# deepomicslab/PALACE

Measured on AMD Instinct MI355X. Metric: contigs/sec eref+generate_graph+matching, 1M-contig synth, 1/2/4/8 GPU, higher is better.
Workload: dtype u32

## Files before the change

palace_amd/csrc/common.hpp:

```cpp
#pragma once
#include <hip/hip_runtime.h>
#include <cstdarg>
#include <cstdint>
#include <cstdio>
#include <cstring>
#include <vector>

#include "../../include/palace_hip.h"

namespace palace {

void set_error(const char *fmt, ...);

#define PALACE_HIP_TRY(expr)                                                                    \
    do {                                                                                        \
        hipError_t e__ = (expr);                                                                \
        if (e__ != hipSuccess) {                                                                \
            palace::set_error("%s failed: %s (%s:%d)", #expr, hipGetErrorString(e__), __FILE__, \
                              __LINE__);                                                        \
            return PALACE_EHIP;                                                                 \
        }                                                                                       \
    } while (0)

#define PALACE_REQUIRE(cond, msg)                                  \
    do {                                                           \
        if (!(cond)) {                                             \
            palace::set_error("%s: %s", __func__, msg);            \
            return PALACE_EINVAL;                                  \
        }                                                          \
    } while (0)

constexpr int kWave = 64;
constexpr int kCUs = 256;
constexpr size_t kPlaneBytes = 1ull << 29;
constexpr size_t kPlaneWords = 1ull << 27;

struct CoderMasks {
    uint32_t m[3][3];
};

struct Workspace {
    void *ptr = nullptr;
    size_t bytes = 0;
};

}

namespace palace {
struct MatchScratch;
void free_match_scratch(MatchScratch *m);
}

struct palace_ctx {
    int device = 0;
    hipStream_t stream = nullptr;
    bool owns_stream = true;
    hipEvent_t ev0 = nullptr, ev1 = nullptr;
    uint32_t key_buckets[4] = {~0u, ~0u, ~0u, ~0u};
    std::vector<hipEvent_t> marks;
    bool coder_set = false;
    palace::CoderMasks masks{};
    uint32_t *plane[3] = {nullptr, nullptr, nullptr};
    bool planes_external = false;
    bool want_final = false;
    bool final_only = false;
    bool table_clean = false;
    int64_t keys_counted = 0;
    const struct palace_eref_probe_index *probe_ix = nullptr;
    const struct palace_eref_probe_index *c0_hits_ix = nullptr;
    uint32_t hits_mask = 0;
    int probe_all_sets = 0;
    bool sent_scattered = false;
    int64_t scan_ref_lo = 0, scan_ref_hi = 0;
    const void *counts_ptr = nullptr;
    bool planeless = false;
    int count_mode = 0;
    int64_t bin_cap_override = 0;
    int64_t slab_override = 0;
    palace::Workspace ws;
    bool ws_grown = false;
    palace::Workspace pin;
    palace::MatchScratch *match_scratch = nullptr;
    int64_t graph_border = -1;
    const void *graph_border_cands = nullptr;
    int64_t graph_border_n = -1;
    int match_grid = 0;
    bool match_two_word_keys = false;
    int match_iters = 0;
    uint64_t *d_small = nullptr;
};

namespace palace {
int ensure_workspace(palace_ctx *ctx, size_t bytes);
int ensure_pinned(palace_ctx *ctx, size_t bytes);
int ensure_table(palace_ctx *ctx);
}
```

palace_amd/csrc/decomp.hip:

```cpp
#include "decomp.hpp"

#include <algorithm>

namespace palace {

namespace {

constexpr uint64_t kNoKey = ~0ull;
constexpr uint64_t kClosed = 0;
constexpr int kStampShift = 42;
constexpr int kPackedShift = 52, kPackedStamps = 1 << (64 - kPackedShift);
constexpr uint64_t kLenMask = (1ull << 40) - 1;


__device__ __forceinline__ uint64_t wave_incl_scan(uint64_t v, int lane)
{
#pragma unroll
    for (int d = 1; d < 64; d <<= 1) {
        const uint64_t u = __shfl_up(v, d);
        if (lane >= d) v += u;
    }
    return v;
}

constexpr int kMaxWaves = 16;

__device__ void scan_partials_body(const uint64_t *__restrict__ in, int64_t n, uint64_t *__restrict__ partials, int blk, int nblk)
{
    __shared__ uint64_t part[kMaxWaves];
    const int64_t chunk = (n + nblk - 1) / nblk;
    const int64_t a = min(n, static_cast<int64_t>(blk) * chunk), e = min(n, a + chunk);
    uint64_t s = 0;
    for (int64_t i = a + threadIdx.x; i < e; i += blockDim.x) s += in[i];
    const int lane = threadIdx.x & 63, waves = static_cast<int>(blockDim.x >> 6);
    s = wave_incl_scan(s, lane);
    if (lane == 63) part[threadIdx.x >> 6] = s;
    __syncthreads();
    if (threadIdx.x == 0) {
        uint64_t t = 0;
        for (int w = 0; w < waves; w++) t += part[w];
        partials[blk] = t;
    }
    __syncthreads();
}

__device__ void scan_prefix_body(uint64_t *__restrict__ partials, int n_parts, uint64_t *__restrict__ total)
{
    __shared__ uint64_t part[kMaxWaves];
    const int lane = threadIdx.x & 63, wv = threadIdx.x >> 6;
    const uint64_t x = static_cast<int>(threadIdx.x) < n_parts ? partials[threadIdx.x] : 0;
    const uint64_t incl = wave_incl_scan(x, lane);
    if (lane == 63) part[wv] = incl;
    __syncthreads();
    uint64_t before = 0;
    for (int w = 0; w < wv; w++) before += part[w];
    if (static_cast<int>(threadIdx.x) < n_parts) partials[threadIdx.x] = before + incl - x;
    if (threadIdx.x == blockDim.x - 1) *total = before + incl;
    __syncthreads();
}

__device__ void scan_apply_body(const uint64_t *__restrict__ in, uint64_t *__restrict__ out, int64_t n, const uint64_t *__restrict__ partials,
                                int blk, int nblk)
{
    __shared__ uint64_t part[kMaxWaves];
    const int64_t chunk = (n + nblk - 1) / nblk;
    const int64_t a = min(n, static_cast<int64_t>(blk) * chunk), e = min(n, a + chunk);
    const int lane = threadIdx.x & 63, wv = threadIdx.x >> 6, waves = static_cast<int>(blockDim.x >> 6);
    uint64_t carry = partials[blk];
    for (int64_t base = a; base < e; base += blockDim.x) {
        const int64_t i = base + threadIdx.x;
        const uint64_t x = i < e ? in[i] : 0;
        const uint64_t incl = wave_incl_scan(x, lane);
        if (lane == 63) part[wv] = incl;
        __syncthreads();
        uint64_t before = 0, all = 0;
        for (int w = 0; w < waves; w++) { if (w < wv) before += part[w]; all += part[w]; }
        if (i < e) out[i] = carry + before + incl - x;
        carry += all;
        __syncthreads();
    }
}

__global__ __launch_bounds__(kDecompBlock) void scan_partials_kernel(const uint64_t *__restrict__ in, const int32_t *__restrict__ n_dev,
                                                                     uint64_t *__restrict__ partials)
{
    scan_partials_body(in, *n_dev, partials, static_cast<int>(blockIdx.x), static_cast<int>(gridDim.x));
}
__global__ __launch_bounds__(kDecompBlock) void scan_prefix_kernel(uint64_t *__restrict__ partials, int n_parts, uint64_t *__restrict__ total)
{
    scan_prefix_body(partials, n_parts, total);
}
__global__ __launch_bounds__(kDecompBlock) void scan_apply_kernel(const uint64_t *__restrict__ in, uint64_t *__restrict__ out,
                                                                  const int32_t *__restrict__ n_dev, const uint64_t *__restrict__ partials)
{
    scan_apply_body(in, out, *n_dev, partials, static_cast<int>(blockIdx.x), static_cast<int>(gridDim.x));
}

struct Span { int tid, n; };
__device__ __forceinline__ Span whole_grid() { return Span{static_cast<int>(blockIdx.x * blockDim.x + threadIdx.x), static_cast<int>(gridDim.x * blockDim.x)}; }

__device__ void ph_init(const DecompBufs &b, Span T, int64_t comp_cap, int64_t vert_cap, int n_flags, int allow_packed)
{
    DecompState *st = b.st;
    const int V = st->V;
    for (int i = T.tid; i < V; i += T.n) { b.bo_hi[i] = kNoKey; b.bi_hi[i] = kNoKey; b.on_path[i] = 0; }
    for (int i = T.tid; i < n_flags; i += T.n) b.changed[i] = 0;
    if (T.tid == 0) {
        st->n_comp = 0; st->n_vert = 0; st->comp_cap = comp_cap; st->vert_cap = vert_cap;
        st->unsettled = 0; st->overflow = 0; st->bad = 0; st->dead = 0; st->scan_total = 0; st->alive_after = 0;
        st->packed = (allow_packed && b.kc && b.pack_bad && *b.pack_bad == 0) ? 1u : 0u;
        if (comp_cap >= 0) b.o_off[0] = 0;
    }
}

__device__ void ph_round_begin(const DecompBufs &b, Span T, int reset_left)
{
    const int V = b.st->V;
    if (!reset_left && b.st->dead) return;
    if (T.tid == 0) { b.st->alive_after = 0; if (reset_left) b.st->dead = 0; }
    const int64_t E = b.st->E;
    for (int64_t e = T.tid; e < E; e += T.n) b.done[e] = 0;
    const bool packed = b.st->packed != 0;
    for (int i = T.tid; i < V; i += T.n) {
        const int s = i >> 1;
        const int64_t l = reset_left ? 1 : b.left[s];
        if (reset_left && !(i & 1)) b.left[s] = 1;
        b.alive[i] = l > 0;
        b.next[i] = -1; b.prev[i] = -1;
        b.bo_hi[i] = b.bi_hi[i] = l > 0 ? kNoKey : kClosed;
        if (!packed) { b.bo_lo[i] = kNoKey; b.bo_lo[V + i] = kNoKey; b.bi_lo[i] = kNoKey; b.bi_lo[V + i] = kNoKey; }
        b.len_a[i] = 0;
    }
}

struct IterArgs {
    uint64_t stamp;
    uint64_t stamp_p;
    int parity;
    int prev_flag, flag;
    int unique_hi;
};


__device__ void ph_propose_hi(const DecompBufs &b, Span T, const IterArgs &a)
{
    if (b.st->dead) return;
    if (a.prev_flag >= 0 && !b.changed[a.prev_flag]) return;
    const int64_t E = b.st->E;
    const int V = b.st->V;
    const int other = (a.parity ^ 1) * V;
    const bool packed = b.st->packed != 0;
    for (int64_t e = T.tid; e < E; e += T.n) {
        if (b.done[e]) continue;
        const int u = b.src[e], v = b.dst[e];
        if (b.bi_hi[v] == kClosed) { b.done[e] = 1; continue; }
        const uint64_t k = packed ? (a.stamp_p | b.kc[e]) : (a.stamp | b.khi[e]);
        if (atomicMin(reinterpret_cast<unsigned long long *>(&b.bo_hi[u]), static_cast<unsigned long long>(k)) == kClosed) { b.done[e] = 1; continue; }
        atomicMin(reinterpret_cast<unsigned long long *>(&b.bi_hi[v]), static_cast<unsigned long long>(k));
        if (!a.unique_hi && !packed) { b.bo_lo[other + u] = kNoKey; b.bi_lo[other + v] = kNoKey; }
    }
}

__device__ void ph_propose_lo(const DecompBufs &b, Span T, const IterArgs &a)
{
    if (b.st->dead) return;
    if (a.prev_flag >= 0 && !b.changed[a.prev_flag]) return;
    if (b.st->packed) return;
    const int64_t E = b.st->E;
    const int mine = a.parity * b.st->V;
    for (int64_t e = T.tid; e < E; e += T.n) {
        if (b.done[e]) continue;
        const int u = b.src[e], v = b.dst[e];
        const uint64_t k = a.stamp | b.khi[e], lo = b.klo[e];
        if (b.bo_hi[u] == k) atomicMin(reinterpret_cast<unsigned long long *>(&b.bo_lo[mine + u]), static_cast<unsigned long long>(lo));
        if (b.bi_hi[v] == k) atomicMin(reinterpret_cast<unsigned long long *>(&b.bi_lo[mine + v]), static_cast<unsigned long long>(lo));
    }
}

__device__ void ph_commit_flag(const DecompBufs &b, Span T, const IterArgs &a, volatile unsigned int *took);
__device__ void ph_commit(const DecompBufs &b, Span T, const IterArgs &a)
{
    if (b.st->dead) return;
    if (a.prev_flag >= 0 && !b.changed[a.prev_flag]) return;
    ph_commit_flag(b, T, a, b.changed + a.flag);
}
__device__ void ph_commit_flag(const DecompBufs &b, Span T, const IterArgs &a, volatile unsigned int *took)
{
    bool any = false;
    const int64_t E = b.st->E;
    const int mine = a.parity * b.st->V;
    const bool packed = b.st->packed != 0;
    for (int64_t e = T.tid; e < E; e += T.n) {
        if (b.done[e]) continue;
        const int u = b.src[e], v = b.dst[e];
        const uint64_t k = packed ? (a.stamp_p | b.kc[e]) : (a.stamp | b.khi[e]);
        if (b.bo_hi[u] != k || b.bi_hi[v] != k) continue;
        const uint64_t lo = b.klo[e];
        if (!a.unique_hi && !packed && (b.bo_lo[mine + u] != lo || b.bi_lo[mine + v] != lo)) continue;
        b.next[u] = v; b.prev[v] = u;
        b.nhi[u] = b.khi[e]; b.nlo[u] = lo;
        b.bo_hi[u] = kClosed; b.bi_hi[v] = kClosed;
        b.done[e] = 1;
        any = true;
    }
    if (__syncthreads_or(any) && threadIdx.x == 0) *took = 1u;
}

__device__ void ph_heads(const DecompBufs &b, Span T, int round, int last_flag)
{
    DecompState *st = b.st;
    if (st->dead) return;
    if (T.tid == 0 && last_flag >= 0 && b.changed[last_flag]) st->unsettled = 1;
    const int V = st->V;
    for (int v = T.tid; v < V; v += T.n) {
        if (!b.alive[v] || b.prev[v] >= 0) continue;
        int len = 0, last = v;
        int64_t least = b.left[v >> 1];
        for (int x = v; x >= 0; x = b.next[x]) {
            b.on_path[x] = round + 1;
            last = x;
            len++;
            least = min(least, b.left[x >> 1]);
        }
        const int twin_first = last ^ 1;
        if (v > twin_first) continue;
        const int64_t uses = twin_first == v ? 2 : 1;
        b.len_a[v] = (1ull << 40) | static_cast<uint64_t>(len);
        b.pay[v] = max(static_cast<int64_t>(1), least / uses);
        b.kind[v] = 0;
        b.open_at[v] = 0;
    }
}

__device__ void ph_cycles(const DecompBufs &b, Span T, int round)
{
    const int V = b.st->V;
    if (b.st->dead) return;
    for (int v = T.tid; v < V; v += T.n) {
        if (!b.alive[v] || b.on_path[v] == round + 1) continue;
        int len = 1, twin_least = v ^ 1, worst = 0;
        uint64_t whi = b.nhi[v], wlo = b.nlo[v];
        int64_t least = b.left[v >> 1];
        bool first = true;
        for (int x = b.next[v]; x != v; x = b.next[x]) {
            if (x < v) { first = false; break; }
            twin_least = min(twin_least, x ^ 1);
            const uint64_t hi = b.nhi[x], lo = b.nlo[x];
            if (hi > whi || (hi == whi && lo > wlo)) { whi = hi; wlo = lo; worst = len; }
            least = min(least, b.left[x >> 1]);
            len++;
        }
        if (!first || v > twin_least) continue;
        const int64_t uses = twin_least == v ? 2 : 1;
        b.len_a[v] = (1ull << 40) | static_cast<uint64_t>(len);
        b.pay[v] = max(static_cast<int64_t>(1), least / uses);
        b.kind[v] = 1;
        b.open_at[v] = (worst + 1) % len;
    }
}

__device__ void ph_emit(const DecompBufs &b, Span T, int round, int64_t c0, int64_t v0)
{
    DecompState *st = b.st;
    const int V = st->V;
    if (st->dead) return;
    int64_t alive = 0;
    for (int v = T.tid; v < V; v += T.n) {
        const uint64_t la = b.len_a[v];
        if (!la) continue;
        const int64_t len = static_cast<int64_t>(la & kLenMask);
        const uint64_t p = b.pos[v];
        const int64_t c = c0 + static_cast<int64_t>(p >> 40), at = v0 + static_cast<int64_t>(p & kLenMask);
        const int64_t pay = b.pay[v];
        const bool room = c < st->comp_cap && at + len <= st->vert_cap;
        if (!room) st->overflow = 1;
        else { b.o_off[c] = at; b.o_kind[c] = b.kind[v]; b.o_iter[c] = round; b.o_open[c] = b.open_at[v]; }
        int x = v;
        int64_t still = 0;
        for (int64_t k = 0; k < len; k++) {
            if (room) b.o_verts[at + k] = 2 * b.orig[x >> 1] + (x & 1);
            const int64_t l = b.left[x >> 1];
            b.left[x >> 1] = max(static_cast<int64_t>(0), l - pay);
            still += l - pay > 0;
            x = b.next[x];
        }
        alive += still;
    }
    __shared__ unsigned long long wg_alive;
    if (threadIdx.x == 0) wg_alive = 0;
    __syncthreads();
    if (alive) atomicAdd(&wg_alive, static_cast<unsigned long long>(alive));
    __syncthreads();
    if (threadIdx.x == 0 && wg_alive) atomicAdd(reinterpret_cast<unsigned long long *>(&st->alive_after), wg_alive);
}


__global__ void dec_init_kernel(DecompBufs b, int64_t comp_cap, int64_t vert_cap, int n_flags, int allow_packed) { ph_init(b, whole_grid(), comp_cap, vert_cap, n_flags, allow_packed); }
__global__ void dec_round_begin_kernel(DecompBufs b, int reset_left) { ph_round_begin(b, whole_grid(), reset_left); }
__global__ void dec_propose_hi_kernel(DecompBufs b, IterArgs a) { ph_propose_hi(b, whole_grid(), a); }
__global__ void dec_propose_lo_kernel(DecompBufs b, IterArgs a) { ph_propose_lo(b, whole_grid(), a); }
__global__ void dec_commit_kernel(DecompBufs b, IterArgs a) { ph_commit(b, whole_grid(), a); }
__global__ void dec_heads_kernel(DecompBufs b, int round, int last_flag) { ph_heads(b, whole_grid(), round, last_flag); }
__global__ void dec_cycles_kernel(DecompBufs b, int round) { ph_cycles(b, whole_grid(), round); }
__global__ void dec_emit_kernel(DecompBufs b, int round) { ph_emit(b, whole_grid(), round, b.st->n_comp, b.st->n_vert); }

__global__ void dec_round_end_kernel(DecompBufs b)
{
    DecompState *st = b.st;
    if (blockIdx.x || threadIdx.x || st->dead) return;
    st->dead = st->alive_after == 0;
    st->n_comp += static_cast<int64_t>(st->scan_total >> 40);
    st->n_vert += static_cast<int64_t>(st->scan_total & kLenMask);
    if (st->n_comp <= st->comp_cap) b.o_off[st->n_comp] = st->n_vert;
}

size_t up256(size_t v) { return (v + 255) / 256 * 256; }

struct Carver {
    char *base;
    size_t used = 0;
    template <class T>
    T *take(size_t n)
    {
        T *p = base ? reinterpret_cast<T *>(base + used) : nullptr;
        used += up256(std::max<size_t>(1, n) * sizeof(T));
        return p;
    }
};

size_t carve_all(DecompBufs &b, char *base, int64_t s_cap, int64_t e_cap, int64_t comp_cap, int64_t vert_cap, int rounds, int iters)
{
    Carver c{base};
    const size_t S = static_cast<size_t>(std::max<int64_t>(1, s_cap)), V = 2 * S, E = static_cast<size_t>(std::max<int64_t>(1, e_cap));
    b.st = c.take<DecompState>(1);
    b.src = c.take<int32_t>(E); b.dst = c.take<int32_t>(E);
    b.khi = c.take<uint64_t>(E); b.klo = c.take<uint64_t>(E);
    b.done = c.take<uint8_t>(E);
    b.kc = c.take<uint64_t>(E);
    b.left = c.take<int64_t>(S); b.orig = c.take<int32_t>(S);
    b.next = c.take<int32_t>(V); b.prev = c.take<int32_t>(V); b.on_path = c.take<int32_t>(V); b.open_at = c.take<int32_t>(V);
    b.nhi = c.take<uint64_t>(V); b.nlo = c.take<uint64_t>(V);
    b.bo_hi = c.take<uint64_t>(V); b.bi_hi = c.take<uint64_t>(V);
    b.bo_lo = c.take<uint64_t>(2 * V); b.bi_lo = c.take<uint64_t>(2 * V);
    b.len_a = c.take<uint64_t>(V); b.pos = c.take<uint64_t>(V);
    b.pay = c.take<int64_t>(V);
    b.alive = c.take<uint8_t>(V); b.kind = c.take<uint8_t>(V);
    b.partials = c.take<uint64_t>(kDecompGrid + 1);
    b.changed = c.take<uint32_t>(static_cast<size_t>(rounds) * static_cast<size_t>(iters));
    b.o_off = c.take<int64_t>(static_cast<size_t>(comp_cap) + 1);
    b.o_verts = c.take<int32_t>(static_cast<size_t>(vert_cap));
    b.o_iter = c.take<int32_t>(static_cast<size_t>(comp_cap));
    b.o_open = c.take<int32_t>(static_cast<size_t>(comp_cap));
    b.o_kind = c.take<uint8_t>(static_cast<size_t>(comp_cap));
    return c.used;
}

}

size_t decomp_bytes(int64_t s_cap, int64_t e_cap, int64_t comp_cap, int64_t vert_cap, int rounds, int iters)
{
    DecompBufs tmp;
    return carve_all(tmp, nullptr, s_cap, e_cap, comp_cap, vert_cap, rounds, iters);
}

void decomp_carve(DecompBufs &b, char *base, int64_t s_cap, int64_t e_cap, int64_t comp_cap, int64_t vert_cap, int rounds, int iters)
{
    carve_all(b, base, s_cap, e_cap, comp_cap, vert_cap, rounds, iters);
}

int scan_u64(palace_ctx *ctx, const uint64_t *in, uint64_t *out, const int32_t *n_dev, uint64_t *partials, uint64_t *total_dev)
{
    hipLaunchKernelGGL(scan_partials_kernel, dim3(kDecompGrid), dim3(kDecompBlock), 0, ctx->stream, in, n_dev, partials);
    hipLaunchKernelGGL(scan_prefix_kernel, dim3(1), dim3(kDecompBlock), 0, ctx->stream, partials, kDecompGrid, total_dev);
    hipLaunchKernelGGL(scan_apply_kernel, dim3(kDecompGrid), dim3(kDecompBlock), 0, ctx->stream, in, out, n_dev, partials);
    PALACE_HIP_TRY(hipGetLastError());
    return PALACE_OK;
}

namespace {

const dim3 kBlock(kDecompBlock);
constexpr int kWideGridDefault = 2048;
inline dim3 wide_grid(const palace_ctx *ctx) { return dim3(ctx->match_grid > 0 ? ctx->match_grid : kWideGridDefault); }

void enqueue_iterations(palace_ctx *ctx, const DecompBufs &b, int first, int n, uint64_t *count, int flag0, bool unique_hi)
{
    for (int k = 0; k < n; k++) {
        IterArgs a{((1ull << 21) - 1 - *count) << kStampShift, static_cast<uint64_t>((kPackedStamps - 1 - *count) & (kPackedStamps - 1)) << kPackedShift,
                   (first + k) & 1, k ? flag0 + k - 1 : -1, flag0 + k, unique_hi ? 1 : 0};
        (*count)++;
        hipLaunchKernelGGL(dec_propose_hi_kernel, wide_grid(ctx), kBlock, 0, ctx->stream, b, a);
        if (!unique_hi) hipLaunchKernelGGL(dec_propose_lo_kernel, wide_grid(ctx), kBlock, 0, ctx->stream, b, a);
        hipLaunchKernelGGL(dec_commit_kernel, wide_grid(ctx), kBlock, 0, ctx->stream, b, a);
    }
}

int enqueue_read_off(palace_ctx *ctx, const DecompBufs &b, int round, int last_flag)
{
    hipLaunchKernelGGL(dec_heads_kernel, wide_grid(ctx), kBlock, 0, ctx->stream, b, round, last_flag);
    hipLaunchKernelGGL(dec_cycles_kernel, wide_grid(ctx), kBlock, 0, ctx->stream, b, round);
    int rc = scan_u64(ctx, b.len_a, b.pos, &b.st->V, b.partials, &b.st->scan_total);
    if (rc) return rc;
    hipLaunchKernelGGL(dec_emit_kernel, wide_grid(ctx), kBlock, 0, ctx->stream, b, round);
    hipLaunchKernelGGL(dec_round_end_kernel, dim3(1), dim3(64), 0, ctx->stream, b);
    PALACE_HIP_TRY(hipGetLastError());
    return PALACE_OK;
}

}

int decomp_begin(palace_ctx *ctx, const DecompBufs &b, int rounds, int64_t comp_cap, int64_t vert_cap)
{
    PALACE_REQUIRE(rounds >= 1 && rounds <= kMaxRounds, "round count out of range");
    static_assert(kDecompGrid <= kDecompBlock, "scan_prefix_kernel scans the block sums with one workgroup");
    const int allow_packed = !ctx->match_two_word_keys && static_cast<int64_t>(rounds) * kMaxIters < kPackedStamps ? 1 : 0;
    hipLaunchKernelGGL(dec_init_kernel, wide_grid(ctx), kBlock, 0, ctx->stream, b, comp_cap, vert_cap, rounds * kMaxIters, allow_packed);
    PALACE_HIP_TRY(hipGetLastError());
    return PALACE_OK;
}

int decomp_rounds(palace_ctx *ctx, const DecompBufs &b, int t0, int t1, int rounds, int aggressive, int iters, bool unique_hi,
                  uint64_t *count)
{
    PALACE_REQUIRE(0 <= t0 && t0 <= t1 && t1 <= rounds && rounds <= kMaxRounds && iters >= 1 && iters <= kMaxIters, "round / iteration count out of range");
    for (int t = t0; t < t1; t++) {
        hipLaunchKernelGGL(dec_round_begin_kernel, wide_grid(ctx), kBlock, 0, ctx->stream, b, (aggressive && t == rounds - 1) ? 1 : 0);
        enqueue_iterations(ctx, b, 0, iters, count, t * kMaxIters, unique_hi);
        int rc = enqueue_read_off(ctx, b, t, t * kMaxIters + iters - 1);
        if (rc) return rc;
    }
    PALACE_HIP_TRY(hipGetLastError());
    return PALACE_OK;
}

int decomp_run_checked(palace_ctx *ctx, const DecompBufs &b, int rounds, int aggressive, bool unique_hi, int64_t comp_cap,
                       int64_t vert_cap, int64_t max_iterations)
{
    PALACE_REQUIRE(rounds >= 1 && rounds <= kMaxRounds, "round count out of range");
    constexpr int kBatch = 16;
    hipLaunchKernelGGL(dec_init_kernel, wide_grid(ctx), kBlock, 0, ctx->stream, b, comp_cap, vert_cap, kBatch, 0);
    uint64_t count = 0;
    for (int t = 0; t < rounds; t++) {
        hipLaunchKernelGGL(dec_round_begin_kernel, wide_grid(ctx), kBlock, 0, ctx->stream, b, (aggressive && t == rounds - 1) ? 1 : 0);
        for (int first = 0;; first += kBatch) {
            PALACE_HIP_TRY(hipMemsetAsync(b.changed, 0, kBatch * sizeof(uint32_t), ctx->stream));
            enqueue_iterations(ctx, b, first, kBatch, &count, 0, unique_hi);
            uint32_t last = 0;
            PALACE_HIP_TRY(hipMemcpyAsync(&last, b.changed + kBatch - 1, sizeof last, hipMemcpyDeviceToHost, ctx->stream));
            PALACE_HIP_TRY(hipStreamSynchronize(ctx->stream));
            if (!last) break;
            if (static_cast<int64_t>(count) > max_iterations || count + kBatch >= (1ull << 21)) {
                set_error("matching: no fixed point after %llu iterations", static_cast<unsigned long long>(count));
                return PALACE_ESTATE;
            }
        }
        PALACE_HIP_TRY(hipMemsetAsync(b.changed, 0, kBatch * sizeof(uint32_t), ctx->stream));
        int rc = enqueue_read_off(ctx, b, t, kBatch - 1);
        if (rc) return rc;
    }
    return PALACE_OK;
}

int decomp_group(palace_ctx *ctx, const DecompBufs &b, DecompRun &run, int rounds, int aggressive, bool unique_hi)
{
    const int first = kFirstGroupRounds;
    const int t0 = run.next_round, t1 = std::min(rounds, t0 + (t0 == 0 ? first : kRoundsPerGroup));
    for (int t = t0; t < t1; t++) {
        const int iters = ctx->match_iters > 0 ? std::min(ctx->match_iters, kMaxIters) : (t == 0 ? kFirstRoundIters : kLaterRoundIters);
        int rc = decomp_rounds(ctx, b, t, t + 1, rounds, aggressive, iters, unique_hi, &run.count);
        if (rc) return rc;
    }
    run.next_round = t1;
    return PALACE_OK;
}

int decomp_finish(palace_ctx *ctx, const DecompBufs &b, DecompRun &run, int rounds, int aggressive, bool unique_hi, int64_t comp_cap,
                  int64_t vert_cap, int64_t max_iterations, DecompState *h_state, const std::function<int()> &reset_left)
{
    for (;;) {
        PALACE_HIP_TRY(hipMemcpyAsync(h_state, b.st, sizeof *h_state, hipMemcpyDeviceToHost, ctx->stream));
        PALACE_HIP_TRY(hipStreamSynchronize(ctx->stream));
        if (h_state->unsettled) {
            int rc = reset_left();
            if (rc) return rc;
            rc = decomp_run_checked(ctx, b, rounds, aggressive, unique_hi, comp_cap, vert_cap, max_iterations);
            if (rc) return rc;
            PALACE_HIP_TRY(hipMemcpyAsync(h_state, b.st, sizeof *h_state, hipMemcpyDeviceToHost, ctx->stream));
            PALACE_HIP_TRY(hipStreamSynchronize(ctx->stream));
            return PALACE_OK;
        }
        if (run.next_round >= rounds) return PALACE_OK;
        if (h_state->alive_after == 0) {
            if (!aggressive) return PALACE_OK;
            run.next_round = rounds - 1;
        }
        int rc = decomp_group(ctx, b, run, rounds, aggressive, unique_hi);
        if (rc) return rc;
    }
}

}
```

palace_amd/csrc/decomp.hpp:

```cpp
#pragma once
#include <functional>

#include "common.hpp"

struct palace_match_result {
    int64_t n = 0;
    int64_t *off = nullptr;
    int32_t *verts = nullptr, *iter = nullptr, *open_at = nullptr;
    uint8_t *kind = nullptr;
    uint64_t *bare = nullptr;
    int64_t n_bare = 0;
    bool borrowed = false;
    ~palace_match_result();
};

namespace palace {

constexpr int kDecompGrid = 256;
constexpr int kDecompBlock = 256;
constexpr int kMaxRounds = 1024;
constexpr int kMaxIters = 64;

struct DecompState {
    int32_t S, V;
    int64_t E;
    int64_t n_comp, n_vert;
    int64_t comp_cap, vert_cap;
    uint32_t unsettled;
    uint32_t overflow;
    uint32_t bad;
    uint32_t dead;
    uint32_t packed;
    uint64_t scan_total;
    int64_t alive_after;
};

struct DecompBufs {
    DecompState *st = nullptr;
    int32_t *src = nullptr, *dst = nullptr;
    uint64_t *khi = nullptr, *klo = nullptr;
    uint8_t *done = nullptr;
    uint64_t *kc = nullptr;
    const uint32_t *pack_bad = nullptr;
    int64_t *left = nullptr;
    int32_t *orig = nullptr;
    int32_t *next = nullptr, *prev = nullptr, *on_path = nullptr, *open_at = nullptr;
    uint64_t *nhi = nullptr, *nlo = nullptr;
    uint64_t *bo_hi = nullptr, *bi_hi = nullptr;
    uint64_t *bo_lo = nullptr, *bi_lo = nullptr;
    uint64_t *len_a = nullptr, *pos = nullptr;
    int64_t *pay = nullptr;
    uint8_t *alive = nullptr, *kind = nullptr;
    uint64_t *partials = nullptr;
    uint32_t *changed = nullptr;
    int64_t *o_off = nullptr;
    int32_t *o_verts = nullptr, *o_iter = nullptr, *o_open = nullptr;
    uint8_t *o_kind = nullptr;
};

size_t decomp_bytes(int64_t s_cap, int64_t e_cap, int64_t comp_cap, int64_t vert_cap, int rounds, int iters);
void decomp_carve(DecompBufs &b, char *base, int64_t s_cap, int64_t e_cap, int64_t comp_cap, int64_t vert_cap, int rounds, int iters);
constexpr int kFirstRoundIters = 7, kLaterRoundIters = 4, kRoundsPerGroup = 5, kFirstGroupRounds = 5;
int decomp_begin(palace_ctx *ctx, const DecompBufs &b, int rounds, int64_t comp_cap, int64_t vert_cap);
int decomp_rounds(palace_ctx *ctx, const DecompBufs &b, int t0, int t1, int rounds, int aggressive, int iters, bool unique_hi,
                  uint64_t *count);

struct DecompRun { int next_round = 0; uint64_t count = 0; };
int decomp_group(palace_ctx *ctx, const DecompBufs &b, DecompRun &run, int rounds, int aggressive, bool unique_hi);
int decomp_finish(palace_ctx *ctx, const DecompBufs &b, DecompRun &run, int rounds, int aggressive, bool unique_hi, int64_t comp_cap,
                  int64_t vert_cap, int64_t max_iterations, DecompState *h_state, const std::function<int()> &reset_left);

int decomp_run_checked(palace_ctx *ctx, const DecompBufs &b, int rounds, int aggressive, bool unique_hi, int64_t comp_cap,
                       int64_t vert_cap, int64_t max_iterations);

int scan_u64(palace_ctx *ctx, const uint64_t *in, uint64_t *out, const int32_t *n_dev, uint64_t *partials, uint64_t *total_dev);

}
```

palace_amd/csrc/filter.hip:

```cpp
#include <algorithm>
#include <cstdlib>
#include <memory>
#include <vector>

#include "common.hpp"
#include "decomp.hpp"

namespace palace {
namespace {

constexpr uint64_t kEmptyKey = ~0ull;
constexpr uint64_t kWeightTop = 1ull << 40;

struct FilterState {
    int32_t n_segs, S_f, n_sel, n_resc;
    int64_t n_edges, n_junc, n_kept2, n_kept3, n_arcs;
    int64_t n_static, n_dyn;
    int64_t n_path_arcs;
    uint32_t bad, pack_bad;
    uint64_t scan_total;
};
enum : uint32_t { kBadPathToken = 1, kBadNoSeg = 2, kBadEdgeBound = 4, kBadArcTable = 8 };

struct ArcTable {
    uint64_t *key;
    unsigned long long *w;
    uint32_t *backed;
    uint64_t mask;
    int64_t *list, list_cap;
};

struct PathArcs {
    uint64_t *key;
    int32_t *idx;
    uint64_t mask;
    int32_t *u, *v;
    int32_t *arc_of;
    int64_t n, cap;
};

struct F {
    FilterState *fs;
    int32_t n_segs, min_count;
    const uint8_t *seed;
    const int32_t *tlen, *rank, *name_len;
    int32_t *by_rank;
    int64_t n_paths;
    const int64_t *path_off;
    const int32_t *path_tok;
    uint8_t *core, *sel, *near, *resc, *seg_flags, *edge_flags, *has_arc;
    int32_t *fid, *contig_of;
    uint64_t *scan_in, *scan_out;
    int64_t edge_bound;
    ArcTable t;
    PathArcs pa;
    int32_t *arc_u, *arc_v;
    unsigned long long *arc_w;
    uint8_t *arc_backed;
    int64_t arc_cap;
    int use_paths;
    uint64_t *bare;
};

__device__ __forceinline__ int gtid() { return static_cast<int>(blockIdx.x * blockDim.x + threadIdx.x); }
__device__ __forceinline__ int gsize() { return static_cast<int>(gridDim.x * blockDim.x); }

__global__ void st4_by_rank_kernel(F f)
{
    for (int s = gtid(); s < f.n_segs; s += gsize()) f.by_rank[f.rank[s]] = s;
}

__global__ void st4_begin_kernel(F f, const int64_t *__restrict__ d_n_edges, int64_t call_bound)
{
    for (int s = gtid(); s < f.n_segs; s += gsize()) {
        const uint8_t c = f.seed[s] != 0 && f.tlen[s] > 0;
        f.core[s] = c; f.sel[s] = c; f.near[s] = 0; f.resc[s] = 0;
    }
    if (gtid() == 0) {
        FilterState *fs = f.fs;
        const int64_t n = *d_n_edges;
        fs->n_segs = f.n_segs; fs->S_f = 0; fs->n_sel = 0; fs->n_resc = 0;
        const int64_t bound = call_bound < f.edge_bound ? call_bound : f.edge_bound;
        fs->n_edges = n < 0 ? 0 : (n > bound ? bound : n);
        fs->n_junc = 0; fs->n_kept2 = 0; fs->n_kept3 = 0; fs->n_arcs = 0; fs->n_static = 0; fs->n_dyn = 0;
        fs->bad = n > bound ? kBadEdgeBound : 0u;
        fs->pack_bad = 0;
        fs->scan_total = 0;
    }
}

__device__ __forceinline__ int64_t edge_total(const palace_graph_edge &e)
{
    return static_cast<int64_t>(e.counts[0]) + e.counts[1] + e.counts[2] + e.counts[3];
}

__global__ void st4_pass2_kernel(F f, const palace_graph_edge *__restrict__ edges)
{
    const int64_t n = f.fs->n_edges;
    int64_t juncs = 0, kept = 0;
    for (int64_t i = gtid(); i < n; i += gsize()) {
        const palace_graph_edge e = edges[i];
        uint8_t fl = 0;
        if (edge_total(e) >= f.min_count) {
            fl = 1; juncs++;
            if (e.left == e.right || f.core[e.left] || f.core[e.right]) {
                fl |= 2; kept++;
                f.near[e.left] = 1; f.near[e.right] = 1;
                f.sel[e.left] = 1; f.sel[e.right] = 1;
            }
        }
        f.edge_flags[i] = fl;
    }
    if (juncs) atomicAdd(reinterpret_cast<unsigned long long *>(&f.fs->n_junc), static_cast<unsigned long long>(juncs));
    if (kept) atomicAdd(reinterpret_cast<unsigned long long *>(&f.fs->n_kept2), static_cast<unsigned long long>(kept));
}

__global__ void st4_pass3_kernel(F f, const palace_graph_edge *__restrict__ edges)
{
    const int64_t n = f.fs->n_edges;
    int64_t kept = 0;
    for (int64_t i = gtid(); i < n; i += gsize()) {
        const uint8_t fl = f.edge_flags[i];
        if (!(fl & 1)) continue;
        const palace_graph_edge e = edges[i];
        if (f.core[e.left] || f.near[e.left] || f.core[e.right] || f.near[e.right]) {
            f.edge_flags[i] = fl | 4;
            if (!(fl & 2)) kept++;
            f.sel[e.left] = 1; f.sel[e.right] = 1;
        }
    }
    if (kept) atomicAdd(reinterpret_cast<unsigned long long *>(&f.fs->n_kept3), static_cast<unsigned long long>(kept));
}

__global__ void st4_paths_kernel(F f)
{
    for (int64_t p = gtid(); p < f.n_paths; p += gsize()) {
        const int64_t a = f.path_off[p], b = f.path_off[p + 1];
        int64_t total = 0, backed = 0;
        bool known = true;
        for (int64_t k = a; k < b; k++) {
            const int32_t t = f.path_tok[k];
            if (t < 0) { known = false; break; }
            const int32_t m = t >> 1;
            total += f.name_len[m];
            if (f.seed[m]) backed += f.name_len[m];
        }
        if (!known) { atomicOr(&f.fs->bad, kBadPathToken); continue; }
        if (backed > 0 && (static_cast<double>(backed) / static_cast<double>(total) >= 0.5 || backed > 2000))
            for (int64_t k = a; k < b; k++) f.resc[f.path_tok[k] >> 1] = 1;
    }
}

__global__ void st4_order_kernel(F f)
{
    for (int r = gtid(); r < f.n_segs; r += gsize()) {
        const int s = f.by_rank[r];
        const bool sel = f.sel[s], resc = f.resc[s] && !sel;
        if (resc && f.tlen[s] <= 0) atomicOr(&f.fs->bad, kBadNoSeg);
        f.scan_in[r] = (sel ? (1ull << 32) : 0ull) | (resc ? 1ull : 0ull);
    }
}

__global__ void st4_ids_kernel(F f)
{
    FilterState *fs = f.fs;
    const int32_t n_sel = static_cast<int32_t>(fs->scan_total >> 32), n_resc = static_cast<int32_t>(fs->scan_total & 0xffffffffu);
    for (int r = gtid(); r < f.n_segs; r += gsize()) {
        const int s = f.by_rank[r];
        const uint64_t in = f.scan_in[r], before = f.scan_out[r];
        int32_t id = -1;
        if (in >> 32) id = static_cast<int32_t>(before >> 32);
        else if (in & 1) id = n_sel + static_cast<int32_t>(before & 0xffffffffu);
        f.fid[s] = id;
        if (id >= 0) { f.contig_of[id] = s; f.has_arc[id] = 0; }
        f.seg_flags[s] = static_cast<uint8_t>((in >> 32 ? 1 : 0) | (in & 1 ? 2 : 0) | (f.core[s] ? 4 : 0));
    }
    if (gtid() == 0) { fs->n_sel = n_sel; fs->n_resc = n_resc; fs->S_f = n_sel + n_resc; }
}

__device__ __forceinline__ uint64_t mix(uint64_t x)
{
    x ^= x >> 33; x *= 0xff51afd7ed558ccdull; x ^= x >> 33; x *= 0xc4ceb9fe1a85ec53ull; x ^= x >> 33;
    return x;
}

__device__ void path_arc_insert(const F &f, int32_t u, int32_t v)
{
    const PathArcs &pa = f.pa;
    const uint64_t key = (static_cast<uint64_t>(static_cast<uint32_t>(u)) << 32) | static_cast<uint32_t>(v);
    uint64_t s = mix(key) & pa.mask;
    for (uint64_t probes = 0; probes <= pa.mask; probes++) {
        const uint64_t cur = pa.key[s];
        if (cur == key) return;
        if (cur == kEmptyKey) {
            const uint64_t old = atomicCAS(reinterpret_cast<unsigned long long *>(&pa.key[s]), kEmptyKey, key);
            if (old == kEmptyKey) {
                const int64_t at = static_cast<int64_t>(atomicAdd(reinterpret_cast<unsigned long long *>(&f.fs->n_path_arcs), 1ull));
                if (at < pa.cap) { pa.u[at] = u; pa.v[at] = v; pa.idx[s] = static_cast<int32_t>(at); }
                return;
            }
            if (old == key) return;
        }
        s = (s + 1) & pa.mask;
    }
}
__global__ void st4_path_arcs_kernel(F f)
{
    for (int64_t p = gtid(); p < f.n_paths; p += gsize()) {
        int32_t before = -1;
        for (int64_t k = f.path_off[p]; k < f.path_off[p + 1]; k++) {
            const int32_t here = f.path_tok[k];
            if (before >= 0 && here >= 0) {
                path_arc_insert(f, before, here);
                if ((here ^ 1) != before) path_arc_insert(f, here ^ 1, before ^ 1);
            }
            before = here;
        }
    }
}
__device__ __forceinline__ int32_t path_arc_find(const PathArcs &pa, int32_t u, int32_t v)
{
    const uint64_t key = (static_cast<uint64_t>(static_cast<uint32_t>(u)) << 32) | static_cast<uint32_t>(v);
    uint64_t s = mix(key) & pa.mask;
    for (;;) {
        const uint64_t cur = pa.key[s];
        if (cur == key) return pa.idx[s];
        if (cur == kEmptyKey) return -1;
        s = (s + 1) & pa.mask;
    }
}

__global__ __launch_bounds__(kDecompBlock) void st4_arcs_static_kernel(F f)
{
    __shared__ uint32_t wave_n[kDecompBlock / 64];
    __shared__ long long block_base;
    const PathArcs &pa = f.pa;
    const int lane = threadIdx.x & 63, wave = threadIdx.x >> 6;
    for (int64_t p0 = static_cast<int64_t>(blockIdx.x) * blockDim.x; p0 < pa.n; p0 += static_cast<int64_t>(gridDim.x) * blockDim.x) {
        const int64_t p = p0 + threadIdx.x;
        int32_t fu = -1, fv = -1;
        if (p < pa.n) {
            const int32_t cu = pa.u[p] >> 1, cv = pa.v[p] >> 1;
            if ((f.seg_flags[cu] & 3) && (f.seg_flags[cv] & 3)) { fu = f.fid[cu]; fv = f.fid[cv]; }
        }
        const bool in = fu >= 0 && fv >= 0;
        const unsigned long long m = __ballot(in);
        if (lane == 0) wave_n[wave] = static_cast<uint32_t>(__popcll(m));
        __syncthreads();
        if (threadIdx.x == 0) {
            uint32_t total = 0;
            for (int w = 0; w < kDecompBlock / 64; w++) { const uint32_t c = wave_n[w]; wave_n[w] = total; total += c; }
            block_base = total ? static_cast<long long>(atomicAdd(reinterpret_cast<unsigned long long *>(&f.fs->n_static), static_cast<unsigned long long>(total))) : 0ll;
        }
        __syncthreads();
        if (p < pa.n) {
            int32_t at = -1;
            if (in) {
                const int64_t slot = block_base + wave_n[wave] + __popcll(m & ((1ull << lane) - 1));
                if (slot < f.arc_cap) {
                    at = static_cast<int32_t>(slot);
                    f.arc_u[at] = 2 * fu + (pa.u[p] & 1); f.arc_v[at] = 2 * fv + (pa.v[p] & 1);
                    f.arc_w[at] = 0; f.arc_backed[at] = 1;
                } else atomicOr(&f.fs->bad, kBadArcTable);
            }
            pa.arc_of[p] = at;
        }
        __syncthreads();
    }
}

__device__ void bump_arc(const F &f, int32_t cu, int32_t cv, int32_t u, int32_t v, int64_t w)
{
    if (f.use_paths) {
        const int32_t p = path_arc_find(f.pa, cu, cv);
        if (p >= 0) {
            const int32_t at = f.pa.arc_of[p];
            if (at >= 0) { atomicAdd(&f.arc_w[at], static_cast<unsigned long long>(w)); return; }
        }
    }
    const ArcTable &t = f.t;
    const uint64_t key = (static_cast<uint64_t>(static_cast<uint32_t>(u)) << 32) | static_cast<uint32_t>(v);
    uint64_t s = mix(key) & t.mask;
    for (uint64_t probes = 0;; probes++) {
        if (probes > t.mask) { atomicOr(&f.fs->bad, kBadArcTable); return; }
        const uint64_t cur = t.key[s];
        if (cur == key) break;
        if (cur == kEmptyKey) {
            const uint64_t old = atomicCAS(reinterpret_cast<unsigned long long *>(&t.key[s]), kEmptyKey, key);
            if (old == kEmptyKey) {
                const int64_t at = static_cast<int64_t>(atomicAdd(reinterpret_cast<unsigned long long *>(&f.fs->n_dyn), 1ull));
                if (at < t.list_cap) t.list[at] = static_cast<int64_t>(s);
                else atomicOr(&f.fs->bad, kBadArcTable);
                break;
            }
            if (old == key) break;
        }
        s = (s + 1) & t.mask;
    }
    if (w) atomicAdd(&t.w[s], static_cast<unsigned long long>(w));
}

__global__ void st4_arcs_juncs_kernel(F f, const palace_graph_edge *__restrict__ edges)
{
    const int64_t n = f.fs->n_edges;
    for (int64_t i = gtid(); i < n; i += gsize()) {
        if (!(f.edge_flags[i] & 6)) continue;
        const palace_graph_edge e = edges[i];
        const int64_t w = min(edge_total(e), static_cast<int64_t>(kWeightTop - 1));
        const int32_t cu = 2 * e.left + (e.oL & 1), cv = 2 * e.right + (e.oR & 1);
        const int32_t u = 2 * f.fid[e.left] + (e.oL & 1), v = 2 * f.fid[e.right] + (e.oR & 1);
        bump_arc(f, cu, cv, u, v, w);
        if ((v ^ 1) != u) bump_arc(f, cv ^ 1, cu ^ 1, v ^ 1, u ^ 1, w);
    }
}

__global__ void st4_arcs_dyn_kernel(F f)
{
    FilterState *fs = f.fs;
    const int64_t n_static = min(fs->n_static, f.arc_cap), n = min(fs->n_dyn, f.t.list_cap);
    for (int64_t a = gtid(); a < n; a += gsize()) {
        const int64_t s = f.t.list[a];
        const uint64_t key = f.t.key[s];
        const int64_t at = n_static + a;
        if (at < f.arc_cap) {
            f.arc_u[at] = static_cast<int32_t>(key >> 32); f.arc_v[at] = static_cast<int32_t>(key & 0xffffffffu);
            f.arc_w[at] = f.t.w[s]; f.arc_backed[at] = 0;
        } else atomicOr(&fs->bad, kBadArcTable);
        f.t.key[s] = kEmptyKey; f.t.w[s] = 0;
    }
    if (gtid() == 0) fs->n_arcs = min(n_static + n, f.arc_cap);
}

__global__ void st4_arc_keys_kernel(F f, DecompBufs b)
{
    const int64_t n = min(f.fs->n_static, f.arc_cap) + min(f.fs->n_dyn, f.t.list_cap);
    for (int64_t a = gtid(); a < n && a < f.arc_cap; a += gsize()) {
        const int32_t u = f.arc_u[a], v = f.arc_v[a];
        const uint64_t w = min(static_cast<uint64_t>(f.arc_w[a]), kWeightTop - 1);
        b.khi[a] = ((kWeightTop - w) << 1) | (f.arc_backed[a] ? 0u : 1u);
        const uint64_t key = (static_cast<uint64_t>(static_cast<uint32_t>(u)) << 32) | static_cast<uint32_t>(v);
        const uint64_t twin = (static_cast<uint64_t>(static_cast<uint32_t>(v ^ 1)) << 32) | static_cast<uint32_t>(u ^ 1);
        const uint64_t cls = min(key, twin);
        b.klo[a] = (cls << 1) | (key != cls ? 1u : 0u);
        f.has_arc[u >> 1] = 1; f.has_arc[v >> 1] = 1;
    }
}

__global__ void st4_sub_in_kernel(F f)
{
    const int n = f.fs->S_f;
    for (int i = gtid(); i < n; i += gsize()) f.scan_in[i] = f.has_arc[i];
}

__global__ void st4_sub_kernel(F f, DecompBufs b, const int32_t *__restrict__ cn)
{
    FilterState *fs = f.fs;
    const int n = fs->S_f;
    const int32_t n_sub = static_cast<int32_t>(fs->scan_total);
    for (int i = gtid(); i < n; i += gsize()) {
        if (!f.has_arc[i]) continue;
        const int32_t sub = static_cast<int32_t>(f.scan_out[i]);
        b.orig[sub] = i;
        b.left[sub] = max(1, cn[f.contig_of[i]]);
    }
    const int64_t n_arcs = min(fs->n_arcs, f.arc_cap);
    const int vbits = 32 - __clz(max(1, 2 * n_sub - 1)), wbits = min(40, 51 - 2 * vbits);
    const uint64_t wmax = wbits > 0 ? (1ull << wbits) - 1 : 0;
    if (gtid() == 0 && wbits <= 0) fs->pack_bad = 1;
    for (int64_t a = gtid(); a < n_arcs; a += gsize()) {
        const int32_t u = f.arc_u[a], v = f.arc_v[a];
        const int32_t su = 2 * static_cast<int32_t>(f.scan_out[u >> 1]) + (u & 1), sv = 2 * static_cast<int32_t>(f.scan_out[v >> 1]) + (v & 1);
        b.src[a] = su;
        b.dst[a] = sv;
        if (wbits > 0) {
            const uint64_t w = f.arc_w[a];
            if (w > wmax) atomicOr(&fs->pack_bad, 1u);
            const uint64_t key = (static_cast<uint64_t>(su) << vbits) | static_cast<uint32_t>(sv);
            const uint64_t twin = (static_cast<uint64_t>(sv ^ 1) << vbits) | static_cast<uint32_t>(su ^ 1);
            b.kc[a] = ((wmax - min(w, wmax)) << (2 * vbits + 1)) | (static_cast<uint64_t>(f.arc_backed[a] ? 0u : 1u) << (2 * vbits)) | min(key, twin);
        }
    }
    if (gtid() == 0) { b.st->S = n_sub; b.st->V = 2 * n_sub; b.st->E = n_arcs; }
}

__global__ void st4_left_kernel(F f, DecompBufs b, const int32_t *__restrict__ cn)
{
    const int n = f.fs->S_f;
    for (int i = gtid(); i < n; i += gsize())
        if (f.has_arc[i]) b.left[static_cast<int32_t>(f.scan_out[i])] = max(1, cn[f.contig_of[i]]);
}

__global__ void st4_bare_kernel(F f)
{
    const int n = f.fs->S_f, words = (n + 63) / 64;
    for (int w = gtid(); w < words; w += gsize()) {
        uint64_t bits = 0;
        for (int k = 0; k < 64 && w * 64 + k < n; k++)
            if (!f.has_arc[w * 64 + k]) bits |= 1ull << k;
        f.bare[w] = bits;
    }
}

size_t up(size_t v) { return (v + 255) / 256 * 256; }
uint64_t pow2_at_least(uint64_t v) { uint64_t p = 1024; while (p < v) p <<= 1; return p; }

template <class T>
T *carve(char *&p, size_t n)
{
    T *r = reinterpret_cast<T *>(p);
    p += up(std::max<size_t>(1, n) * sizeof(T));
    return r;
}

}
}

struct palace_stage04 {
    palace::F f{};
    palace::DecompBufs b{};
    char *fixed = nullptr;
    char *grown = nullptr;
    size_t grown_bytes = 0;
    int64_t n_tok = 0, edge_bound = 0, s_cap = 0, e_cap = 0, comp_cap = 0, vert_cap = 0;
    int rounds = 0, aggressive = 0, last_rounds = 0;
    palace::DecompRun run;
    bool filtered = false, matched = false;
    const int32_t *d_cn = nullptr;
    char *pin = nullptr;
    size_t pin_bytes = 0;
    palace::FilterState *h_fs = nullptr;
    palace::DecompState *h_ds = nullptr;
    palace_match_result res;
    int32_t *h_contig_of = nullptr;
};

using namespace palace;

namespace {

const dim3 kG(1024), kB(kDecompBlock);

int grow_pinned(palace_ctx *ctx, palace_stage04 *s, size_t bytes)
{
    if (s->pin_bytes >= bytes) return PALACE_OK;
    if (s->pin) { PALACE_HIP_TRY(hipStreamSynchronize(ctx->stream)); PALACE_HIP_TRY(hipHostFree(s->pin)); s->pin = nullptr; s->pin_bytes = 0; }
    const size_t want = bytes + bytes / 4 + (1 << 16);
    hipError_t e = hipHostMalloc(reinterpret_cast<void **>(&s->pin), want, hipHostMallocDefault);
    if (e != hipSuccess) { set_error("stage04: hipHostMalloc(%zu) failed: %s", want, hipGetErrorString(e)); return PALACE_ENOMEM; }
    s->pin_bytes = want;
    return PALACE_OK;
}

int grow_device(palace_ctx *ctx, palace_stage04 *s, int64_t edge_bound, int rounds)
{
    const int64_t e_dyn = 2 * edge_bound + 16;
    const int64_t e_cap = e_dyn + s->f.pa.n + 16;
    const int64_t s_cap = std::min<int64_t>(s->f.n_segs, e_cap);
    const int64_t comp_cap = static_cast<int64_t>(rounds) * s_cap + 16, vert_cap = 2 * comp_cap;
    const uint64_t slots = pow2_at_least(2 * static_cast<uint64_t>(e_dyn));
    const size_t dec = decomp_bytes(s_cap, e_cap, comp_cap, vert_cap, rounds, kMaxIters);
    const size_t bytes = up(static_cast<size_t>(edge_bound) + 1) + up(slots * 8) * 2 + up(static_cast<size_t>(e_dyn) * 8) +
                         2 * up(static_cast<size_t>(e_cap) * 4) + up(static_cast<size_t>(e_cap) * 8) + up(static_cast<size_t>(e_cap)) + dec + 8192;
    if (s->grown_bytes < bytes || s->edge_bound < edge_bound || s->rounds < rounds) {
        if (s->grown) { PALACE_HIP_TRY(hipStreamSynchronize(ctx->stream)); PALACE_HIP_TRY(hipFree(s->grown)); s->grown = nullptr; s->grown_bytes = 0; }
        hipError_t e = hipMalloc(reinterpret_cast<void **>(&s->grown), bytes);
        if (e != hipSuccess) { set_error("stage04: hipMalloc(%zu) failed: %s", bytes, hipGetErrorString(e)); return PALACE_ENOMEM; }
        s->grown_bytes = bytes;
        char *p = s->grown;
        s->f.edge_flags = carve<uint8_t>(p, static_cast<size_t>(edge_bound) + 1);
        s->f.t.key = carve<uint64_t>(p, slots);
        s->f.t.w = carve<unsigned long long>(p, slots);
        s->f.t.backed = nullptr;
        s->f.t.mask = slots - 1;
        s->f.t.list = carve<int64_t>(p, static_cast<size_t>(e_dyn));
        s->f.t.list_cap = e_dyn;
        s->f.arc_u = carve<int32_t>(p, static_cast<size_t>(e_cap));
        s->f.arc_v = carve<int32_t>(p, static_cast<size_t>(e_cap));
        s->f.arc_w = carve<unsigned long long>(p, static_cast<size_t>(e_cap));
        s->f.arc_backed = carve<uint8_t>(p, static_cast<size_t>(e_cap));
        s->f.arc_cap = e_cap;
        decomp_carve(s->b, p, s_cap, e_cap, comp_cap, vert_cap, rounds, kMaxIters);
        s->b.pack_bad = &s->f.fs->pack_bad;
        PALACE_HIP_TRY(hipMemsetAsync(s->f.t.key, 0xff, slots * 8, ctx->stream));
        PALACE_HIP_TRY(hipMemsetAsync(s->f.t.w, 0, slots * 8, ctx->stream));
        s->edge_bound = edge_bound; s->s_cap = s_cap; s->e_cap = e_cap; s->comp_cap = comp_cap; s->vert_cap = vert_cap; s->rounds = rounds;
    }
    s->f.edge_bound = s->edge_bound;
    return PALACE_OK;
}

}

extern "C" {

int palace_stage04_create(palace_ctx *ctx, const palace_stage04_inputs *in, palace_stage04 **out)
{
    PALACE_REQUIRE(ctx && in && out, "null argument");
    PALACE_REQUIRE(in->n_segs >= 0 && in->n_segs < (1 << 30) && in->n_paths >= 0 && in->min_count >= 0, "bad size");
    PALACE_REQUIRE(in->n_segs == 0 || (in->seed && in->tlen && in->rank && in->name_len), "null per-contig array");
    PALACE_REQUIRE(in->n_paths == 0 || (in->path_off && in->path_tok), "null path arrays");
    PALACE_HIP_TRY(hipSetDevice(ctx->device));
    const size_t n = static_cast<size_t>(in->n_segs);
    const int64_t n_tok = in->n_paths ? in->path_off[in->n_paths] : 0;
    PALACE_REQUIRE(n_tok >= 0 && (in->n_paths == 0 || in->path_off[0] == 0), "path offsets must start at 0 and ascend");
    int64_t n_pairs = 0;
    for (int64_t k = 0; k < in->n_paths; k++) {
        const int64_t len = in->path_off[k + 1] - in->path_off[k];
        PALACE_REQUIRE(len >= 0 && in->path_off[k + 1] <= n_tok, "path offsets must start at 0 and ascend");
        n_pairs += len > 1 ? len - 1 : 0;
    }
    for (int32_t i = 0; i < in->n_segs; i++) PALACE_REQUIRE(in->rank[i] >= 0 && in->rank[i] < in->n_segs, "rank out of range");
    for (int64_t k = 0; k < n_tok; k++) PALACE_REQUIRE(in->path_tok[k] < 2 * static_cast<int64_t>(in->n_segs), "path token out of range");
    std::unique_ptr<palace_stage04> s(new palace_stage04());
    const int64_t pa_cap = 2 * n_pairs + 16;
    const uint64_t pa_slots = pow2_at_least(2 * static_cast<uint64_t>(pa_cap));
    const size_t bytes = up(sizeof(FilterState)) + up(n) * 8 + up(n * 4) * 6 + up(n * 8) * 2 + up((static_cast<size_t>(in->n_paths) + 1) * 8) +
                         up(static_cast<size_t>(n_tok) * 4 + 4) + up((n + 63) / 64 * 8 + 8) + up(pa_slots * 8) + up(pa_slots * 4) +
                         3 * up(static_cast<size_t>(pa_cap) * 4) + 16384;
    hipError_t e = hipMalloc(reinterpret_cast<void **>(&s->fixed), bytes);
    if (e != hipSuccess) { set_error("stage04: hipMalloc(%zu) failed: %s", bytes, hipGetErrorString(e)); return PALACE_ENOMEM; }
    char *p = s->fixed;
    F &f = s->f;
    f.fs = carve<FilterState>(p, 1);
    f.n_segs = in->n_segs; f.min_count = in->min_count; f.n_paths = in->n_paths;
    uint8_t *seed = carve<uint8_t>(p, n);
    f.core = carve<uint8_t>(p, n); f.sel = carve<uint8_t>(p, n); f.near = carve<uint8_t>(p, n); f.resc = carve<uint8_t>(p, n);
    f.seg_flags = carve<uint8_t>(p, n); f.has_arc = carve<uint8_t>(p, n);
    int32_t *tlen = carve<int32_t>(p, n), *rank = carve<int32_t>(p, n), *name_len = carve<int32_t>(p, n);
    f.by_rank = carve<int32_t>(p, n); f.fid = carve<int32_t>(p, n); f.contig_of = carve<int32_t>(p, n);
    f.scan_in = carve<uint64_t>(p, n); f.scan_out = carve<uint64_t>(p, n);
    int64_t *path_off = carve<int64_t>(p, static_cast<size_t>(in->n_paths) + 1);
    int32_t *path_tok = carve<int32_t>(p, static_cast<size_t>(n_tok) + 1);
    f.bare = carve<uint64_t>(p, (n + 63) / 64 + 1);
    f.pa.key = carve<uint64_t>(p, pa_slots); f.pa.idx = carve<int32_t>(p, pa_slots); f.pa.mask = pa_slots - 1;
    f.pa.u = carve<int32_t>(p, static_cast<size_t>(pa_cap)); f.pa.v = carve<int32_t>(p, static_cast<size_t>(pa_cap));
    f.pa.arc_of = carve<int32_t>(p, static_cast<size_t>(pa_cap));
    f.pa.cap = pa_cap; f.pa.n = 0;
    f.seed = seed; f.tlen = tlen; f.rank = rank; f.name_len = name_len; f.path_off = path_off; f.path_tok = path_tok;
    s->n_tok = n_tok;
    auto fail = [&](hipError_t err) {
        set_error("stage04: upload failed: %s", hipGetErrorString(err));
        (void)hipFree(s->fixed);
        return PALACE_EHIP;
    };
    hipStream_t st = ctx->stream;
    if (n) {
        if ((e = hipMemcpyAsync(seed, in->seed, n, hipMemcpyHostToDevice, st)) != hipSuccess) return fail(e);
        if ((e = hipMemcpyAsync(tlen, in->tlen, n * 4, hipMemcpyHostToDevice, st)) != hipSuccess) return fail(e);
        if ((e = hipMemcpyAsync(rank, in->rank, n * 4, hipMemcpyHostToDevice, st)) != hipSuccess) return fail(e);
        if ((e = hipMemcpyAsync(name_len, in->name_len, n * 4, hipMemcpyHostToDevice, st)) != hipSuccess) return fail(e);
    }
    if (in->n_paths) {
        if ((e = hipMemcpyAsync(path_off, in->path_off, (static_cast<size_t>(in->n_paths) + 1) * 8, hipMemcpyHostToDevice, st)) != hipSuccess) return fail(e);
        if (n_tok && (e = hipMemcpyAsync(path_tok, in->path_tok, static_cast<size_t>(n_tok) * 4, hipMemcpyHostToDevice, st)) != hipSuccess) return fail(e);
    } else if ((e = hipMemsetAsync(path_off, 0, 8, st)) != hipSuccess) return fail(e);
    hipLaunchKernelGGL(st4_by_rank_kernel, kG, kB, 0, st, f);
    if ((e = hipMemsetAsync(f.fs, 0, sizeof(FilterState), st)) != hipSuccess) return fail(e);
    if ((e = hipMemsetAsync(f.pa.key, 0xff, pa_slots * 8, st)) != hipSuccess) return fail(e);
    hipLaunchKernelGGL(st4_path_arcs_kernel, kG, kB, 0, st, f);
    FilterState h_fs{};
    if ((e = hipMemcpyAsync(&h_fs, f.fs, sizeof h_fs, hipMemcpyDeviceToHost, st)) != hipSuccess) return fail(e);
    if ((e = hipStreamSynchronize(st)) != hipSuccess) return fail(e);
    if (h_fs.n_path_arcs > pa_cap) { (void)hipFree(s->fixed); set_error("stage04: path arc table too small"); return PALACE_ESTATE; }
    f.pa.n = h_fs.n_path_arcs;
    e = hipHostMalloc(reinterpret_cast<void **>(&s->h_fs), up(sizeof(FilterState)) + up(sizeof(DecompState)), hipHostMallocDefault);
    if (e != hipSuccess) { (void)hipFree(s->fixed); set_error("stage04: hipHostMalloc failed: %s", hipGetErrorString(e)); return PALACE_ENOMEM; }
    s->h_ds = reinterpret_cast<DecompState *>(reinterpret_cast<char *>(s->h_fs) + up(sizeof(FilterState)));
    s->res.borrowed = true;
    *out = s.release();
    return PALACE_OK;
}

int palace_stage04_destroy(palace_ctx *ctx, palace_stage04 *s)
{
    if (!s) return PALACE_OK;
    if (ctx) { (void)hipSetDevice(ctx->device); (void)hipStreamSynchronize(ctx->stream); }
    if (s->fixed) (void)hipFree(s->fixed);
    if (s->grown) (void)hipFree(s->grown);
    if (s->pin) (void)hipHostFree(s->pin);
    if (s->h_fs) (void)hipHostFree(s->h_fs);
    delete s;
    return PALACE_OK;
}

int palace_stage04_reserve(palace_ctx *ctx, palace_stage04 *s, int64_t edge_bound)
{
    PALACE_REQUIRE(ctx && s && edge_bound >= 0, "bad argument");
    PALACE_HIP_TRY(hipSetDevice(ctx->device));
    return grow_device(ctx, s, std::max<int64_t>(edge_bound, s->edge_bound), std::max(s->rounds, 11));
}

int palace_stage04_filter(palace_ctx *ctx, palace_stage04 *s, const palace_graph_edge *d_edges, const int64_t *d_n_edges,
                          int64_t edge_bound)
{
    PALACE_REQUIRE(ctx && s && d_n_edges && edge_bound >= 0, "bad argument");
    PALACE_REQUIRE(edge_bound == 0 || d_edges, "null edge array");
    PALACE_HIP_TRY(hipSetDevice(ctx->device));
    int rc = grow_device(ctx, s, std::max<int64_t>(edge_bound, s->edge_bound), std::max(s->rounds, 11));
    if (rc) return rc;
    rc = [&]() -> int {
        const F &f = s->f;
        hipStream_t st = ctx->stream;
        hipLaunchKernelGGL(st4_begin_kernel, kG, kB, 0, st, f, d_n_edges, edge_bound);
        hipLaunchKernelGGL(st4_pass2_kernel, kG, kB, 0, st, f, d_edges);
        hipLaunchKernelGGL(st4_pass3_kernel, kG, kB, 0, st, f, d_edges);
        hipLaunchKernelGGL(st4_paths_kernel, kG, kB, 0, st, f);
        hipLaunchKernelGGL(st4_order_kernel, kG, kB, 0, st, f);
        PALACE_HIP_TRY(hipGetLastError());
        int rc2 = scan_u64(ctx, f.scan_in, f.scan_out, &f.fs->n_segs, s->b.partials, &f.fs->scan_total);
        if (rc2) return rc2;
        hipLaunchKernelGGL(st4_ids_kernel, kG, kB, 0, st, f);
        PALACE_HIP_TRY(hipGetLastError());
        return PALACE_OK;
    }();
    if (rc) return rc;
    s->filtered = true;
    s->matched = false;
    return PALACE_OK;
}

static int enqueue_match(palace_ctx *ctx, palace_stage04 *s, const palace_graph_edge *d_edges, bool use_paths)
{
    s->f.use_paths = use_paths ? 1 : 0;
    const F &f = s->f;
    hipStream_t st = ctx->stream;
    if (use_paths) hipLaunchKernelGGL(st4_arcs_static_kernel, kG, kB, 0, st, f);
    hipLaunchKernelGGL(st4_arcs_juncs_kernel, kG, kB, 0, st, f, d_edges);
    hipLaunchKernelGGL(st4_arcs_dyn_kernel, kG, kB, 0, st, f);
    hipLaunchKernelGGL(st4_arc_keys_kernel, kG, kB, 0, st, f, s->b);
    hipLaunchKernelGGL(st4_sub_in_kernel, kG, kB, 0, st, f);
    PALACE_HIP_TRY(hipGetLastError());
    int rc = scan_u64(ctx, f.scan_in, f.scan_out, &f.fs->S_f, s->b.partials, &f.fs->scan_total);
    if (rc) return rc;
    hipLaunchKernelGGL(st4_sub_kernel, kG, kB, 0, st, f, s->b, s->d_cn);
    hipLaunchKernelGGL(st4_bare_kernel, kG, kB, 0, st, f);
    PALACE_HIP_TRY(hipGetLastError());
    return PALACE_OK;
}

int palace_stage04_match(palace_ctx *ctx, palace_stage04 *s, const palace_graph_edge *d_edges, const int32_t *d_cn,
                         int32_t iterations, int32_t aggressive, int32_t use_paths)
{
    PALACE_REQUIRE(ctx && s && d_cn && iterations >= 1, "bad argument");
    PALACE_REQUIRE(s->filtered, "palace_stage04_filter has not run");
    const int rounds = iterations + (aggressive ? 1 : 0);
    PALACE_REQUIRE(rounds <= kMaxRounds, "too many iterations");
    PALACE_REQUIRE(rounds <= s->rounds, "more rounds than the filter call reserved room for (at most 10 iterations + aggressive)");
    PALACE_HIP_TRY(hipSetDevice(ctx->device));
    s->d_cn = d_cn; s->aggressive = aggressive ? 1 : 0;
    s->f.use_paths = use_paths ? 1 : 0;
    int rc = enqueue_match(ctx, s, d_edges, use_paths != 0);
    if (rc) return rc;
    s->run = DecompRun{};
    if ((rc = decomp_begin(ctx, s->b, rounds, s->comp_cap, s->vert_cap))) return rc;
    if ((rc = decomp_group(ctx, s->b, s->run, rounds, s->aggressive, false))) return rc;
    PALACE_HIP_TRY(hipMemcpyAsync(s->h_fs, s->f.fs, sizeof(FilterState), hipMemcpyDeviceToHost, ctx->stream));
    s->rounds = std::max(s->rounds, rounds);
    s->matched = true;
    s->last_rounds = rounds;
    return PALACE_OK;
}

static int check_filter_state(const FilterState &fs)
{
    if (fs.bad & kBadPathToken) { set_error("stage04: contigs.paths names an unknown contig id (filter_graph.py:138 raises)"); return PALACE_EINVAL; }
    if (fs.bad & kBadNoSeg) { set_error("stage04: contigs.paths rescues a contig without SEG line (filter_graph.py:257 raises)"); return PALACE_EINVAL; }
    if (fs.bad & kBadEdgeBound) { set_error("stage04: more edges on the device than the bound given to palace_stage04_filter"); return PALACE_EINVAL; }
    if (fs.bad & kBadArcTable) { set_error("stage04: arc table full"); return PALACE_ESTATE; }
    return PALACE_OK;
}

int palace_stage04_counts(palace_ctx *ctx, palace_stage04 *s, int64_t counts[8])
{
    PALACE_REQUIRE(ctx && s && counts && s->filtered, "bad argument");
    PALACE_HIP_TRY(hipMemcpyAsync(s->h_fs, s->f.fs, sizeof(FilterState), hipMemcpyDeviceToHost, ctx->stream));
    PALACE_HIP_TRY(hipStreamSynchronize(ctx->stream));
    const FilterState &fs = *s->h_fs;
    int rc = check_filter_state(fs);
    if (rc) return rc;
    counts[0] = fs.n_edges; counts[1] = fs.n_junc; counts[2] = fs.n_kept2; counts[3] = fs.n_kept3;
    counts[4] = fs.n_sel; counts[5] = fs.n_resc; counts[6] = s->matched ? fs.n_arcs : -1; counts[7] = fs.S_f;
    return PALACE_OK;
}

int palace_stage04_flags(palace_ctx *ctx, palace_stage04 *s, uint8_t *h_seg_flags, uint8_t *h_edge_flags, int64_t n_edges)
{
    PALACE_REQUIRE(ctx && s && s->filtered && n_edges >= 0 && n_edges <= s->edge_bound, "bad argument");
    if (h_seg_flags && s->f.n_segs)
        PALACE_HIP_TRY(hipMemcpyAsync(h_seg_flags, s->f.seg_flags, static_cast<size_t>(s->f.n_segs), hipMemcpyDeviceToHost, ctx->stream));
    if (h_edge_flags && n_edges)
        PALACE_HIP_TRY(hipMemcpyAsync(h_edge_flags, s->f.edge_flags, static_cast<size_t>(n_edges), hipMemcpyDeviceToHost, ctx->stream));
    PALACE_HIP_TRY(hipStreamSynchronize(ctx->stream));
    return PALACE_OK;
}

int palace_stage04_result(palace_ctx *ctx, palace_stage04 *s, palace_match_result **out, const int32_t **contig_of_out,
                          int64_t *n_segs_filtered_out)
{
    PALACE_REQUIRE(ctx && s && out, "null argument");
    PALACE_REQUIRE(s->matched, "palace_stage04_match has not run");
    PALACE_HIP_TRY(hipSetDevice(ctx->device));
    hipStream_t st = ctx->stream;
    const int rounds = s->last_rounds;
    auto reset_left = [&]() -> int {
        hipLaunchKernelGGL(st4_left_kernel, kG, kB, 0, st, s->f, s->b, s->d_cn);
        PALACE_HIP_TRY(hipGetLastError());
        return PALACE_OK;
    };
    int rc = decomp_finish(ctx, s->b, s->run, rounds, s->aggressive, false, s->comp_cap, s->vert_cap, 2 * s->e_cap + 64, s->h_ds, reset_left);
    if (rc) return rc;
    rc = check_filter_state(*s->h_fs);
    if (rc) return rc;
    const DecompState &ds = *s->h_ds;
    if (ds.overflow || ds.n_comp > s->comp_cap || ds.n_vert > s->vert_cap) { set_error("stage04: component arrays too small"); return PALACE_ESTATE; }
    const size_t nc = static_cast<size_t>(ds.n_comp), nv = static_cast<size_t>(ds.n_vert), sf = static_cast<size_t>(s->h_fs->S_f);
    const size_t words = (sf + 63) / 64;
    rc = grow_pinned(ctx, s, up((nc + 1) * 8) + up(nv * 4 + 4) + 2 * up(nc * 4 + 4) + up(nc + 1) + up(words * 8 + 8) + up(sf * 4 + 4));
    if (rc) return rc;
    char *p = s->pin;
    palace_match_result &r = s->res;
    r.off = carve<int64_t>(p, nc + 1); r.verts = carve<int32_t>(p, nv + 1); r.iter = carve<int32_t>(p, nc + 1);
    r.open_at = carve<int32_t>(p, nc + 1); r.kind = carve<uint8_t>(p, nc + 1); r.bare = carve<uint64_t>(p, words + 1);
    s->h_contig_of = carve<int32_t>(p, sf + 1);
    PALACE_HIP_TRY(hipMemcpyAsync(r.off, s->b.o_off, (nc + 1) * 8, hipMemcpyDeviceToHost, st));
    if (nv) PALACE_HIP_TRY(hipMemcpyAsync(r.verts, s->b.o_verts, nv * 4, hipMemcpyDeviceToHost, st));
    if (nc) {
        PALACE_HIP_TRY(hipMemcpyAsync(r.iter, s->b.o_iter, nc * 4, hipMemcpyDeviceToHost, st));
        PALACE_HIP_TRY(hipMemcpyAsync(r.open_at, s->b.o_open, nc * 4, hipMemcpyDeviceToHost, st));
        PALACE_HIP_TRY(hipMemcpyAsync(r.kind, s->b.o_kind, nc, hipMemcpyDeviceToHost, st));
    }
    if (words) PALACE_HIP_TRY(hipMemcpyAsync(r.bare, s->f.bare, words * 8, hipMemcpyDeviceToHost, st));
    if (sf) PALACE_HIP_TRY(hipMemcpyAsync(s->h_contig_of, s->f.contig_of, sf * 4, hipMemcpyDeviceToHost, st));
    PALACE_HIP_TRY(hipStreamSynchronize(st));
    r.n = static_cast<int64_t>(nc);
    r.n_bare = static_cast<int64_t>(sf) - ds.S;
    *out = &s->res;
    if (contig_of_out) *contig_of_out = s->h_contig_of;
    if (n_segs_filtered_out) *n_segs_filtered_out = static_cast<int64_t>(sf);
    return PALACE_OK;
}

}
```

palace_amd/csrc/match.hip:

```cpp
#include "common.hpp"
#include "decomp.hpp"
#include <algorithm>
#include <map>
#include <memory>
#include <mutex>
#include <numeric>
#include <thread>

namespace palace {

constexpr int32_t kNone = -1;

struct MatchArgs {
    int32_t n_vertices;
    int64_t n_arcs;
    const int32_t *src, *dst;
    const int64_t *out_off, *in_off;
    const int32_t *out_arcs, *in_arcs;
    const uint8_t *alive;
    int32_t *next, *prev, *next_arc, *want_out, *want_in;
    unsigned int *changed;
};

__global__ void match_propose_kernel(MatchArgs a)
{
    int32_t v = blockIdx.x * blockDim.x + threadIdx.x;
    if (v >= a.n_vertices) return;
    int32_t wo = kNone, wi = kNone;
    if (a.alive[v]) {
        if (a.next[v] == kNone)
            for (int64_t k = a.out_off[v]; k < a.out_off[v + 1]; k++) {
                int32_t e = a.out_arcs[k], h = a.dst[e];
                if (a.alive[h] && a.prev[h] == kNone) { wo = e; break; }
            }
        if (a.prev[v] == kNone)
            for (int64_t k = a.in_off[v]; k < a.in_off[v + 1]; k++) {
                int32_t e = a.in_arcs[k], t = a.src[e];
                if (a.alive[t] && a.next[t] == kNone) { wi = e; break; }
            }
    }
    a.want_out[v] = wo;
    a.want_in[v] = wi;
}

__global__ void match_commit_kernel(MatchArgs a)
{
    int32_t v = blockIdx.x * blockDim.x + threadIdx.x;
    if (v >= a.n_vertices) return;
    int32_t e = a.want_out[v];
    if (e == kNone) return;
    int32_t h = a.dst[e];
    if (a.want_in[h] != e) return;
    a.next[v] = h;
    a.prev[h] = v;
    a.next_arc[v] = e;
    *a.changed = 1u;
}

__global__ void match_init_kernel(MatchArgs a)
{
    int32_t v = blockIdx.x * blockDim.x + threadIdx.x;
    if (v >= a.n_vertices) return;
    a.next[v] = kNone; a.prev[v] = kNone; a.next_arc[v] = kNone;
}

}

using namespace palace;

constexpr int kRoundsPerCheck = 4;

static int enqueue_rounds(palace_ctx *ctx, const MatchArgs &a, int n)
{
    const unsigned blocks = static_cast<unsigned>((a.n_vertices + 255) / 256);
    PALACE_HIP_TRY(hipMemsetAsync(a.changed, 0, 4, ctx->stream));
    for (int k = 0; k < n; k++) {
        hipLaunchKernelGGL(match_propose_kernel, dim3(blocks), dim3(256), 0, ctx->stream, a);
        hipLaunchKernelGGL(match_commit_kernel, dim3(blocks), dim3(256), 0, ctx->stream, a);
    }
    PALACE_HIP_TRY(hipGetLastError());
    return PALACE_OK;
}

extern "C" int palace_match_greedy(palace_ctx *ctx, int32_t n_vertices, int64_t n_arcs, const int32_t *d_src,
                                   const int32_t *d_dst, const int64_t *d_out_off, const int32_t *d_out_arcs,
                                   const int64_t *d_in_off, const int32_t *d_in_arcs, const uint8_t *d_alive,
                                   int32_t *d_next, int32_t *d_prev, int32_t *d_next_arc, int32_t *rounds_out)
{
    PALACE_REQUIRE(ctx && n_vertices >= 0 && n_arcs >= 0, "bad argument");
    if (rounds_out) *rounds_out = 0;
    if (n_vertices == 0) return PALACE_OK;
    PALACE_REQUIRE(d_out_off && d_in_off && d_alive && d_next && d_prev && d_next_arc, "null device pointer");
    PALACE_REQUIRE(n_arcs == 0 || (d_src && d_dst && d_out_arcs && d_in_arcs), "null arc arrays");
    PALACE_REQUIRE(n_arcs < (1ll << 31), "arc ids must fit in int32");
    PALACE_HIP_TRY(hipSetDevice(ctx->device));
    int rc = ensure_workspace(ctx, static_cast<size_t>(n_vertices) * 8 + 256);
    if (rc) return rc;
    MatchArgs a{};
    a.n_vertices = n_vertices; a.n_arcs = n_arcs; a.src = d_src; a.dst = d_dst;
    a.out_off = d_out_off; a.in_off = d_in_off; a.out_arcs = d_out_arcs; a.in_arcs = d_in_arcs;
    a.alive = d_alive; a.next = d_next; a.prev = d_prev; a.next_arc = d_next_arc;
    a.want_out = static_cast<int32_t *>(ctx->ws.ptr);
    a.want_in = a.want_out + n_vertices;
    a.changed = reinterpret_cast<unsigned int *>(ctx->d_small);
    const unsigned blocks = static_cast<unsigned>((n_vertices + 255) / 256);
    hipLaunchKernelGGL(match_init_kernel, dim3(blocks), dim3(256), 0, ctx->stream, a);
    int rounds = 0;
    for (;;) {
        unsigned int changed = 0;
        rc = enqueue_rounds(ctx, a, kRoundsPerCheck);
        if (rc) return rc;
        PALACE_HIP_TRY(hipMemcpyAsync(&changed, ctx->d_small, 4, hipMemcpyDeviceToHost, ctx->stream));
        PALACE_HIP_TRY(hipStreamSynchronize(ctx->stream));
        rounds += kRoundsPerCheck;
        if (!changed) break;
        if (rounds > n_vertices + 2 + kRoundsPerCheck) { set_error("palace_match_greedy: no fixed point"); return PALACE_ESTATE; }
    }
    if (rounds_out) *rounds_out = rounds;
    return PALACE_OK;
}

struct SubResult {
    std::vector<int64_t> off{0};
    std::vector<int32_t> verts, iter, open_at;
    std::vector<uint8_t> kind;
};

namespace palace {

class BlockPool {
public:
    void *take(size_t bytes)
    {
        bytes = std::max<size_t>(bytes, 64);
        {
            std::lock_guard<std::mutex> g(mu_);
            for (size_t i = 0; i < free_.size(); i++)
                if (free_[i].second >= bytes && free_[i].second <= 2 * bytes + (1 << 20)) {
                    void *p = free_[i].first;
                    sizes_[p] = free_[i].second;
                    free_.erase(free_.begin() + i);
                    return p;
                }
        }
        void *p = std::malloc(bytes);
        if (p) { std::lock_guard<std::mutex> g(mu_); sizes_[p] = bytes; }
        return p;
    }
    void give(void *p)
    {
        if (!p) return;
        std::lock_guard<std::mutex> g(mu_);
        const size_t bytes = sizes_[p];
        sizes_.erase(p);
        if (free_.size() < 16) free_.emplace_back(p, bytes);
        else std::free(p);
    }

private:
    std::mutex mu_;
    std::vector<std::pair<void *, size_t>> free_;
    std::map<void *, size_t> sizes_;
};
static BlockPool g_result_pool;

struct MatchScratch {
    std::vector<int32_t> new_id, old_id, ssrc, sdst;
    std::vector<int64_t> sub_copies;
    std::vector<uint64_t> has_arc;
    SubResult sub;
};
void free_match_scratch(MatchScratch *m) { delete m; }

template <class T>
struct Borrowed {
    T &home;
    T v;
    explicit Borrowed(T &h) : home(h), v(std::move(h)) {}
    ~Borrowed() { home = std::move(v); }
    Borrowed(const Borrowed &) = delete;
    Borrowed &operator=(const Borrowed &) = delete;
};

__global__ void iota_keys_kernel(uint64_t *__restrict__ khi, uint64_t *__restrict__ klo, int64_t n)
{
    for (int64_t i = static_cast<int64_t>(blockIdx.x) * blockDim.x + threadIdx.x; i < n; i += static_cast<int64_t>(gridDim.x) * blockDim.x) {
        khi[i] = static_cast<uint64_t>(i);
        klo[i] = 0;
    }
}

}

palace_match_result::~palace_match_result()
{
    if (borrowed) return;
    for (void *p : {(void *)off, (void *)verts, (void *)iter, (void *)open_at, (void *)kind, (void *)bare}) palace::g_result_pool.give(p);
}

static int decompose_core(palace_ctx *ctx, int32_t n_segs, const int64_t *copies, const int32_t *orig, int64_t n_arcs,
                          const int32_t *src, const int32_t *dst, int32_t iterations, int32_t aggressive, SubResult *res)
{
    using namespace palace;
    const int64_t S = n_segs, E = n_arcs;
    const int rounds = iterations + (aggressive ? 1 : 0);
    PALACE_REQUIRE(rounds <= kMaxRounds, "too many iterations");
    int64_t live_rounds = 0;
    for (int64_t s = 0; s < S; s++) live_rounds += std::min<int64_t>(iterations, std::max<int64_t>(1, copies[s]));
    if (aggressive) live_rounds += S;
    const int64_t comp_cap = live_rounds, vert_cap = 2 * live_rounds;
    const size_t dev_bytes = decomp_bytes(S, E, comp_cap, vert_cap, rounds, kMaxIters);
    int rc = ensure_workspace(ctx, dev_bytes);
    if (rc) return rc;
    DecompBufs b;
    decomp_carve(b, static_cast<char *>(ctx->ws.ptr), S, E, comp_cap, vert_cap, rounds, kMaxIters);
    const size_t e4 = (static_cast<size_t>(E) * 4 + 255) / 256 * 256, s8 = (static_cast<size_t>(S) * 8 + 255) / 256 * 256,
                 s4 = (static_cast<size_t>(S) * 4 + 255) / 256 * 256;
    rc = ensure_pinned(ctx, 2 * e4 + s8 + s4 + 512);
    if (rc) return rc;
    char *pin = static_cast<char *>(ctx->pin.ptr);
    int32_t *p_src = reinterpret_cast<int32_t *>(pin), *p_dst = reinterpret_cast<int32_t *>(pin + e4);
    int64_t *p_left = reinterpret_cast<int64_t *>(pin + 2 * e4);
    int32_t *p_orig = reinterpret_cast<int32_t *>(pin + 2 * e4 + s8);
    DecompState *p_st = reinterpret_cast<DecompState *>(pin + 2 * e4 + s8 + s4);
    DecompState *p_back = p_st + 1;
    std::copy(src, src + E, p_src); std::copy(dst, dst + E, p_dst);
    for (int64_t s = 0; s < S; s++) p_left[s] = std::max<int64_t>(1, copies[s]);
    std::copy(orig, orig + S, p_orig);
    std::memset(p_st, 0, sizeof *p_st);
    p_st->S = n_segs; p_st->V = 2 * n_segs; p_st->E = E;
    hipStream_t st = ctx->stream;
    auto upload = [&]() -> int {
        PALACE_HIP_TRY(hipMemcpyAsync(b.st, p_st, sizeof *p_st, hipMemcpyHostToDevice, st));
        if (E) {
            PALACE_HIP_TRY(hipMemcpyAsync(b.src, p_src, static_cast<size_t>(E) * 4, hipMemcpyHostToDevice, st));
            PALACE_HIP_TRY(hipMemcpyAsync(b.dst, p_dst, static_cast<size_t>(E) * 4, hipMemcpyHostToDevice, st));
            hipLaunchKernelGGL(iota_keys_kernel, dim3(kDecompGrid), dim3(kDecompBlock), 0, st, b.khi, b.klo, E);
        }
        PALACE_HIP_TRY(hipMemcpyAsync(b.left, p_left, static_cast<size_t>(S) * 8, hipMemcpyHostToDevice, st));
        PALACE_HIP_TRY(hipMemcpyAsync(b.orig, p_orig, static_cast<size_t>(S) * 4, hipMemcpyHostToDevice, st));
        return PALACE_OK;
    };
    auto fail = [&](int code) { (void)hipStreamSynchronize(st); return code; };
    hipError_t e = hipSuccess;
    if ((rc = upload())) return fail(rc);
    if ((rc = decomp_begin(ctx, b, rounds, comp_cap, vert_cap))) return fail(rc);
    DecompRun run;
    if ((rc = decomp_group(ctx, b, run, rounds, aggressive, true))) return fail(rc);
    auto reset_left = [&]() -> int {
        PALACE_HIP_TRY(hipMemcpyAsync(b.left, p_left, static_cast<size_t>(S) * 8, hipMemcpyHostToDevice, st));
        return PALACE_OK;
    };
    if ((rc = decomp_finish(ctx, b, run, rounds, aggressive, true, comp_cap, vert_cap, 2 * E + 64, p_back, reset_left))) return fail(rc);
    if (p_back->overflow || p_back->n_comp > comp_cap || p_back->n_vert > vert_cap) {
        set_error("decompose: component arrays too small (%lld components, %lld vertices)", (long long)p_back->n_comp, (long long)p_back->n_vert);
        return PALACE_ESTATE;
    }
    const size_t nc = static_cast<size_t>(p_back->n_comp), nv = static_cast<size_t>(p_back->n_vert);
    res->off.resize(nc + 1); res->verts.resize(nv); res->iter.resize(nc); res->open_at.resize(nc); res->kind.resize(nc);
    e = hipMemcpyAsync(res->off.data(), b.o_off, (nc + 1) * 8, hipMemcpyDeviceToHost, st);
    if (e == hipSuccess && nv) e = hipMemcpyAsync(res->verts.data(), b.o_verts, nv * 4, hipMemcpyDeviceToHost, st);
    if (e == hipSuccess && nc) e = hipMemcpyAsync(res->iter.data(), b.o_iter, nc * 4, hipMemcpyDeviceToHost, st);
    if (e == hipSuccess && nc) e = hipMemcpyAsync(res->open_at.data(), b.o_open, nc * 4, hipMemcpyDeviceToHost, st);
    if (e == hipSuccess && nc) e = hipMemcpyAsync(res->kind.data(), b.o_kind, nc, hipMemcpyDeviceToHost, st);
    if (e == hipSuccess) e = hipStreamSynchronize(st);
    if (e != hipSuccess) { set_error("decompose: %s", hipGetErrorString(e)); return fail(PALACE_EHIP); }
    return PALACE_OK;
}

namespace {

void radix_by(const std::vector<uint64_t> &key, std::vector<uint32_t> &perm, std::vector<uint32_t> &tmp)
{
    const size_t n = perm.size();
    uint64_t all_or = 0, all_and = ~0ull;
    for (size_t i = 0; i < n; i++) { all_or |= key[i]; all_and &= key[i]; }
    const uint64_t varying = all_or ^ all_and;
    std::vector<uint32_t> hist(65536);
    for (int shift = 0; shift < 64; shift += 16) {
        if (((varying >> shift) & 0xffffu) == 0) continue;
        std::fill(hist.begin(), hist.end(), 0u);
        for (size_t i = 0; i < n; i++) hist[(key[perm[i]] >> shift) & 0xffffu]++;
        uint32_t run = 0;
        for (auto &h : hist) { const uint32_t c = h; h = run; run += c; }
        for (size_t i = 0; i < n; i++) tmp[hist[(key[perm[i]] >> shift) & 0xffffu]++] = perm[i];
        perm.swap(tmp);
    }
}

}

extern "C" {

int palace_match_arcs_from_edges(const int32_t *cn, int32_t n_segs, const palace_graph_edge *edges, int64_t n_edges,
                                 int32_t min_count, int64_t *copies, int32_t *src, int32_t *dst, int64_t *weight,
                                 int64_t *n_arcs_out)
{
    PALACE_REQUIRE(n_segs >= 0 && n_edges >= 0 && n_arcs_out, "bad argument");
    PALACE_REQUIRE(n_segs == 0 || (cn && copies), "null segment arrays");
    PALACE_REQUIRE(n_edges == 0 || (edges && src && dst && weight), "null edge arrays");
    PALACE_REQUIRE(n_segs < (1 << 30) && n_edges < (1ll << 30), "graph too large for int32 ids");
    for (int32_t s = 0; s < n_segs; s++) copies[s] = std::max(1, cn[s]);
    const uint64_t V = 2ull * static_cast<uint64_t>(n_segs);
    static thread_local std::vector<uint64_t> pair, m_pair, m_cls, m_wkey;
    static thread_local std::vector<int64_t> w, m_w;
    static thread_local std::vector<uint32_t> perm, tmp;
    pair.clear(); w.clear(); m_pair.clear(); m_w.clear();
    pair.reserve(2 * n_edges); w.reserve(2 * n_edges);
    for (int64_t e = 0; e < n_edges; e++) {
        const palace_graph_edge &x = edges[e];
        const int64_t tot = static_cast<int64_t>(x.counts[0]) + x.counts[1] + x.counts[2] + x.counts[3];
        if (tot < min_count) continue;
        PALACE_REQUIRE(x.left >= 0 && x.left < n_segs && x.right >= 0 && x.right < n_segs, "edge endpoint out of range");
        const uint64_t u = 2ull * x.left + (x.oL & 1), v = 2ull * x.right + (x.oR & 1);
        pair.push_back(u * V + v); w.push_back(tot);
        if ((v ^ 1) != u) { pair.push_back((v ^ 1) * V + (u ^ 1)); w.push_back(tot); }
    }
    const size_t n = pair.size();
    perm.resize(n); tmp.resize(n);
    std::iota(perm.begin(), perm.end(), 0u);
    radix_by(pair, perm, tmp);
    m_pair.reserve(n); m_w.reserve(n);
    for (size_t i = 0; i < n; i++) {
        if (!m_pair.empty() && m_pair.back() == pair[perm[i]]) m_w.back() += w[perm[i]];
        else { m_pair.push_back(pair[perm[i]]); m_w.push_back(w[perm[i]]); }
    }
    const size_t m = m_pair.size();
    int64_t w_max = 0;
    for (int64_t x : m_w) w_max = std::max(w_max, x);
    m_cls.resize(m); m_wkey.resize(m);
    for (size_t i = 0; i < m; i++) {
        const uint64_t u = m_pair[i] / V, v = m_pair[i] % V;
        m_cls[i] = std::min(m_pair[i], (v ^ 1) * V + (u ^ 1));
        m_wkey[i] = static_cast<uint64_t>(w_max - m_w[i]);
    }
    perm.resize(m); tmp.resize(m);
    std::iota(perm.begin(), perm.end(), 0u);
    radix_by(m_cls, perm, tmp);
    radix_by(m_wkey, perm, tmp);
    for (size_t i = 0; i < m; i++) {
        const uint64_t p = m_pair[perm[i]];
        src[i] = static_cast<int32_t>(p / V); dst[i] = static_cast<int32_t>(p % V); weight[i] = m_w[perm[i]];
    }
    *n_arcs_out = static_cast<int64_t>(m);
    return PALACE_OK;
}

int palace_match_set_option(palace_ctx *ctx, const char *name, int64_t value)
{
    PALACE_REQUIRE(ctx && name, "null argument");
    if (!std::strcmp(name, "iters_per_round")) {
        PALACE_REQUIRE(value >= 0 && value <= palace::kMaxIters, "iters_per_round out of range");
        ctx->match_iters = static_cast<int>(value);
    } else if (!std::strcmp(name, "one_word_keys")) {
        PALACE_REQUIRE(value == 0 || value == 1, "one_word_keys must be 0 or 1");
        ctx->match_two_word_keys = value == 0;
    } else if (!std::strcmp(name, "decomp_grid")) {
        PALACE_REQUIRE(value >= 0 && value <= 65536, "decomp_grid out of range");
        ctx->match_grid = static_cast<int>(value);
    } else {
        palace::set_error("palace_match_set_option: unknown option '%s'", name);
        return PALACE_EINVAL;
    }
    return PALACE_OK;
}

int palace_match_decompose(palace_ctx *ctx, int32_t n_segs, const int64_t *copies, int64_t n_arcs,
                           const int32_t *src, const int32_t *dst, int32_t iterations, int32_t aggressive,
                           palace_match_result **out)
{
    return palace_match_decompose_ex(ctx, n_segs, copies, n_arcs, src, dst, iterations, aggressive, 0, out);
}

int palace_match_decompose_ex(palace_ctx *ctx, int32_t n_segs, const int64_t *copies, int64_t n_arcs,
                              const int32_t *src, const int32_t *dst, int32_t iterations, int32_t aggressive,
                              int32_t compact, palace_match_result **out)
{
    PALACE_REQUIRE(ctx && out && n_segs >= 0 && n_arcs >= 0 && iterations >= 1, "bad argument");
    PALACE_REQUIRE(n_segs == 0 || copies, "null copies");
    PALACE_REQUIRE(n_arcs == 0 || (src && dst), "null arc arrays");
    PALACE_REQUIRE(n_segs < (1 << 30) && n_arcs < (1ll << 31), "graph too large for int32 ids");
    PALACE_HIP_TRY(hipSetDevice(ctx->device));
    const int32_t V = 2 * n_segs;
    for (int64_t e = 0; e < n_arcs; e++)
        PALACE_REQUIRE(src[e] >= 0 && src[e] < V && dst[e] >= 0 && dst[e] < V, "arc endpoint out of range");
    if (!ctx->match_scratch) ctx->match_scratch = new palace::MatchScratch();
    palace::MatchScratch &ms = *ctx->match_scratch;
    palace::Borrowed<std::vector<int32_t>> b_new(ms.new_id), b_old(ms.old_id), b_ssrc(ms.ssrc), b_sdst(ms.sdst);
    palace::Borrowed<std::vector<int64_t>> b_sc(ms.sub_copies);
    auto &new_id = b_new.v, &old_id = b_old.v, &ssrc = b_ssrc.v, &sdst = b_sdst.v;
    auto &sub_copies = b_sc.v;
    SubResult &sub = ms.sub;
    const size_t n_words = (static_cast<size_t>(n_segs) + 63) / 64;
    palace::Borrowed<std::vector<uint64_t>> b_bits(ms.has_arc);
    auto &has_arc = b_bits.v;
    has_arc.assign(n_words, 0);
    for (int64_t e = 0; e < n_arcs; e++) {
        const int32_t a = src[e] >> 1, b = dst[e] >> 1;
        has_arc[a >> 6] |= 1ull << (a & 63);
        has_arc[b >> 6] |= 1ull << (b & 63);
    }
    new_id.resize(n_words + 1);
    old_id.clear();
    for (size_t w = 0; w < n_words; w++) {
        new_id[w] = static_cast<int32_t>(old_id.size());
        for (uint64_t x = has_arc[w]; x; x &= x - 1) old_id.push_back(static_cast<int32_t>(w * 64 + __builtin_ctzll(x)));
    }
    new_id[n_words] = static_cast<int32_t>(old_id.size());
    auto is_sub = [&](int32_t sg) { return (has_arc[sg >> 6] >> (sg & 63)) & 1ull; };
    auto sub_rank = [&](int32_t sg) {
        if (sg >= n_segs) return new_id[n_words];
        return new_id[sg >> 6] + __builtin_popcountll(has_arc[sg >> 6] & ((1ull << (sg & 63)) - 1));
    };
    const int32_t n_sub = static_cast<int32_t>(old_id.size());
    sub_copies.resize(n_sub);
    for (int32_t k = 0; k < n_sub; k++) sub_copies[k] = copies[old_id[k]];
    ssrc.resize(n_arcs); sdst.resize(n_arcs);
    for (int64_t e = 0; e < n_arcs; e++) {
        ssrc[e] = 2 * sub_rank(src[e] >> 1) + (src[e] & 1);
        sdst[e] = 2 * sub_rank(dst[e] >> 1) + (dst[e] & 1);
    }
    sub.off.assign(1, 0); sub.verts.clear(); sub.iter.clear(); sub.open_at.clear(); sub.kind.clear();
    int rc = n_sub ? decompose_core(ctx, n_sub, sub_copies.data(), old_id.data(), n_arcs, ssrc.data(), sdst.data(), iterations, aggressive, &sub)
                   : PALACE_OK;
    if (rc) return rc;
    const int64_t n_sub_comp = static_cast<int64_t>(sub.kind.size());
    const int last_round = iterations + (aggressive ? 1 : 0) - 1;
    const int64_t n_bare = static_cast<int64_t>(n_segs) - n_sub;
    if (compact) {
        palace_match_result *res = new palace_match_result();
        const int64_t nv = static_cast<int64_t>(sub.verts.size());
        res->off = static_cast<int64_t *>(palace::g_result_pool.take((n_sub_comp + 1) * 8));
        res->kind = static_cast<uint8_t *>(palace::g_result_pool.take(n_sub_comp + 1));
        res->iter = static_cast<int32_t *>(palace::g_result_pool.take((n_sub_comp + 1) * 4));
        res->open_at = static_cast<int32_t *>(palace::g_result_pool.take((n_sub_comp + 1) * 4));
        res->verts = static_cast<int32_t *>(palace::g_result_pool.take((nv + 1) * 4));
        res->bare = static_cast<uint64_t *>(palace::g_result_pool.take((n_words + 1) * 8));
        if (!res->off || !res->kind || !res->iter || !res->open_at || !res->verts || !res->bare) {
            delete res;
            palace::set_error("palace_match_decompose: out of host memory");
            return PALACE_ENOMEM;
        }
        std::copy(sub.off.begin(), sub.off.end(), res->off);
        std::copy(sub.kind.begin(), sub.kind.end(), res->kind);
        std::copy(sub.iter.begin(), sub.iter.end(), res->iter);
        std::copy(sub.open_at.begin(), sub.open_at.end(), res->open_at);
        std::copy(sub.verts.begin(), sub.verts.end(), res->verts);
        for (size_t w = 0; w < n_words; w++) res->bare[w] = ~has_arc[w];
        if (n_segs & 63) res->bare[n_words - 1] &= (1ull << (n_segs & 63)) - 1;
        res->n = n_sub_comp;
        res->n_bare = n_bare;
        *out = res;
        return PALACE_OK;
    }
    const int64_t n_out = n_sub_comp + n_bare * (aggressive && last_round > 0 ? 2 : 1);
    const int64_t nv_out = static_cast<int64_t>(sub.verts.size()) + (n_out - n_sub_comp);
    palace_match_result *res = new palace_match_result();
    res->off = static_cast<int64_t *>(palace::g_result_pool.take((n_out + 1) * 8));
    res->kind = static_cast<uint8_t *>(palace::g_result_pool.take(n_out));
    res->iter = static_cast<int32_t *>(palace::g_result_pool.take(n_out * 4));
    res->open_at = static_cast<int32_t *>(palace::g_result_pool.take(n_out * 4));
    res->verts = static_cast<int32_t *>(palace::g_result_pool.take(nv_out * 4));
    if (!res->off || !res->kind || !res->iter || !res->open_at || !res->verts) {
        delete res;
        palace::set_error("palace_match_decompose: out of host memory");
        return PALACE_ENOMEM;
    }
    int64_t *r_off = res->off;
    int32_t *r_verts = res->verts, *r_iter = res->iter, *r_open = res->open_at;
    uint8_t *r_kind = res->kind;
    r_off[0] = 0;
    auto split = [&](int64_t c) { return (sub.verts[sub.off[c]] + 1) >> 1; };
    auto merge_range = [&](int32_t a, int32_t b, int64_t c_lo, int64_t c_hi, int64_t oc, int64_t ov, int round) {
        int32_t s = a;
        auto bare_until = [&](int32_t until) {
            for (; s < until; s++) {
                if (is_sub(s)) continue;
                r_verts[ov++] = 2 * s;
                r_kind[oc] = 0; r_iter[oc] = round; r_open[oc] = 0;
                r_off[++oc] = ov;
            }
        };
        for (int64_t c = c_lo; c < c_hi; c++) {
            bare_until(std::min<int32_t>(b, split(c)));
            const int64_t len = sub.off[c + 1] - sub.off[c];
            std::copy(sub.verts.begin() + sub.off[c], sub.verts.begin() + sub.off[c + 1], r_verts + ov);
            ov += len;
            r_kind[oc] = sub.kind[c]; r_iter[oc] = sub.iter[c]; r_open[oc] = sub.open_at[c];
            r_off[++oc] = ov;
        }
        bare_until(b);
    };
    int64_t oc = 0, ov = 0, c = 0;
    for (int round = 0; round <= last_round; round++) {
        int64_t c_end = c;
        while (c_end < n_sub_comp && sub.iter[c_end] == round) c_end++;
        const bool bare_round = round == 0 || (aggressive && round == last_round);
        if (!bare_round) {
            merge_range(0, 0, c, c_end, oc, ov, round);
            oc += c_end - c; ov += sub.off[c_end] - sub.off[c];
            c = c_end;
            continue;
        }
        const int n_thr = n_segs >= (1 << 17) ? 4 : 1;
        std::vector<std::thread> pool;
        int64_t c_lo = c;
        for (int k = 0; k < n_thr; k++) {
            const int32_t a = static_cast<int32_t>(static_cast<int64_t>(n_segs) * k / n_thr);
            const int32_t b = static_cast<int32_t>(static_cast<int64_t>(n_segs) * (k + 1) / n_thr);
            int64_t c_hi = c_end;
            if (k + 1 < n_thr) {
                int64_t lo = c_lo, hi = c_end;
                while (lo < hi) { const int64_t mid = (lo + hi) / 2; if (split(mid) < b) lo = mid + 1; else hi = mid; }
                c_hi = lo;
            }
            const int64_t n_sub_in = sub_rank(b) - sub_rank(a);
            const int64_t n_bare_in = (b - a) - n_sub_in;
            if (n_thr == 1) merge_range(a, b, c_lo, c_hi, oc, ov, round);
            else pool.emplace_back(merge_range, a, b, c_lo, c_hi, oc, ov, round);
            oc += n_bare_in + (c_hi - c_lo);
            ov += n_bare_in + (sub.off[c_hi] - sub.off[c_lo]);
            c_lo = c_hi;
        }
        for (auto &t : pool) t.join();
        c = c_end;
    }
    res->n = oc;
    *out = res;
    return PALACE_OK;
}

int64_t palace_match_result_count(const palace_match_result *r) { return r ? r->n : 0; }
const int64_t *palace_match_result_offsets(const palace_match_result *r) { return r ? r->off : nullptr; }
const int32_t *palace_match_result_verts(const palace_match_result *r) { return r ? r->verts : nullptr; }
const uint8_t *palace_match_result_kind(const palace_match_result *r) { return r ? r->kind : nullptr; }
const int32_t *palace_match_result_iter(const palace_match_result *r) { return r ? r->iter : nullptr; }
const int32_t *palace_match_result_open_at(const palace_match_result *r) { return r ? r->open_at : nullptr; }
const uint64_t *palace_match_result_bare(const palace_match_result *r) { return r ? r->bare : nullptr; }
int64_t palace_match_result_bare_count(const palace_match_result *r) { return r ? r->n_bare : 0; }
void palace_match_result_free(palace_match_result *r) { if (r && !r->borrowed) delete r; }

}
```

Before: 111.3 million.

## Run decomposition tail rounds in a single-block kernel over compacted lists

After the first round, the remaining live vertices and arcs are compacted into lists, and the later rounds run inside one 1024-thread block that loops over propose/commit without per-iteration kernel launches or host syncs. The scan drops its separate prefix kernel by folding the partial prefix into the apply kernel. Emit now finishes the round on device with a ticket counter, and a skip_lo/refused path falls back to the checked path. This targets launch and host round-trip overhead for small residual graphs, at the cost of serial single-block work when the tail is large and added fallback complexity.

New measurement: 107.7 million. 3.2% lower.

```diff
diff --git a/palace_amd/csrc/common.hpp b/palace_amd/csrc/common.hpp
--- a/palace_amd/csrc/common.hpp
+++ b/palace_amd/csrc/common.hpp
@@ -87,6 +87,7 @@
     int match_grid = 0;
     bool match_two_word_keys = false;
     int match_iters = 0;
+    int match_tail_cap = -1;
     uint64_t *d_small = nullptr;
 };
 
diff --git a/palace_amd/csrc/decomp.hip b/palace_amd/csrc/decomp.hip
--- a/palace_amd/csrc/decomp.hip
+++ b/palace_amd/csrc/decomp.hip
@@ -44,29 +44,21 @@
     __syncthreads();
 }
 
-__device__ void scan_prefix_body(uint64_t *__restrict__ partials, int n_parts, uint64_t *__restrict__ total)
-{
-    __shared__ uint64_t part[kMaxWaves];
-    const int lane = threadIdx.x & 63, wv = threadIdx.x >> 6;
-    const uint64_t x = static_cast<int>(threadIdx.x) < n_parts ? partials[threadIdx.x] : 0;
-    const uint64_t incl = wave_incl_scan(x, lane);
-    if (lane == 63) part[wv] = incl;
-    __syncthreads();
-    uint64_t before = 0;
-    for (int w = 0; w < wv; w++) before += part[w];
-    if (static_cast<int>(threadIdx.x) < n_parts) partials[threadIdx.x] = before + incl - x;
-    if (threadIdx.x == blockDim.x - 1) *total = before + incl;
-    __syncthreads();
-}
-
 __device__ void scan_apply_body(const uint64_t *__restrict__ in, uint64_t *__restrict__ out, int64_t n, const uint64_t *__restrict__ partials,
-                                int blk, int nblk)
-{
-    __shared__ uint64_t part[kMaxWaves];
+                                int blk, int nblk, uint64_t *__restrict__ total)
+{
+    __shared__ uint64_t part[kMaxWaves], part_all[kMaxWaves];
     const int64_t chunk = (n + nblk - 1) / nblk;
     const int64_t a = min(n, static_cast<int64_t>(blk) * chunk), e = min(n, a + chunk);
     const int lane = threadIdx.x & 63, wv = threadIdx.x >> 6, waves = static_cast<int>(blockDim.x >> 6);
-    uint64_t carry = partials[blk];
+    const uint64_t mine = static_cast<int>(threadIdx.x) < nblk ? partials[threadIdx.x] : 0;
+    const uint64_t front = wave_incl_scan(static_cast<int>(threadIdx.x) < blk ? mine : 0, lane), every = wave_incl_scan(mine, lane);
+    if (lane == 63) { part[wv] = front; part_all[wv] = every; }
+    __syncthreads();
+    uint64_t carry = 0, sum = 0;
+    for (int w = 0; w < waves; w++) { carry += part[w]; sum += part_all[w]; }
+    if (blk == 0 && threadIdx.x == 0) *total = sum;
+    __syncthreads();
     for (int64_t base = a; base < e; base += blockDim.x) {
         const int64_t i = base + threadIdx.x;
         const uint64_t x = i < e ? in[i] : 0;
@@ -86,20 +78,26 @@
 {
     scan_partials_body(in, *n_dev, partials, static_cast<int>(blockIdx.x), static_cast<int>(gridDim.x));
 }
-__global__ __launch_bounds__(kDecompBlock) void scan_prefix_kernel(uint64_t *__restrict__ partials, int n_parts, uint64_t *__restrict__ total)
-{
-    scan_prefix_body(partials, n_parts, total);
-}
 __global__ __launch_bounds__(kDecompBlock) void scan_apply_kernel(const uint64_t *__restrict__ in, uint64_t *__restrict__ out,
-                                                                  const int32_t *__restrict__ n_dev, const uint64_t *__restrict__ partials)
-{
-    scan_apply_body(in, out, *n_dev, partials, static_cast<int>(blockIdx.x), static_cast<int>(gridDim.x));
+                                                                  const int32_t *__restrict__ n_dev, const uint64_t *__restrict__ partials,
+                                                                  uint64_t *__restrict__ total)
+{
+    scan_apply_body(in, out, *n_dev, partials, static_cast<int>(blockIdx.x), static_cast<int>(gridDim.x), total);
 }
 
 struct Span { int tid, n; };
 __device__ __forceinline__ Span whole_grid() { return Span{static_cast<int>(blockIdx.x * blockDim.x + threadIdx.x), static_cast<int>(gridDim.x * blockDim.x)}; }
 
-__device__ void ph_init(const DecompBufs &b, Span T, int64_t comp_cap, int64_t vert_cap, int n_flags, int allow_packed)
+template <bool Listed> __device__ __forceinline__ int n_vertices(const DecompBufs &b) { return Listed ? b.st->tail_nv : b.st->V; }
+template <bool Listed> __device__ __forceinline__ int64_t n_arcs(const DecompBufs &b) { return Listed ? static_cast<int64_t>(b.st->tail_ne) : b.st->E; }
+template <bool Listed> __device__ __forceinline__ int vertex_at(const DecompBufs &b, int j) { return Listed ? b.vlist[j] : j; }
+template <bool Listed> __device__ __forceinline__ int64_t arc_at(const DecompBufs &b, int64_t j) { return Listed ? static_cast<int64_t>(b.alist[j]) : j; }
+template <bool Listed> __device__ __forceinline__ uint64_t slot_word(const uint64_t *p)
+{
+    return Listed ? __hip_atomic_load(p, __ATOMIC_RELAXED, __HIP_MEMORY_SCOPE_AGENT) : *p;
+}
+
+__device__ void ph_init(const DecompBufs &b, Span T, int64_t comp_cap, int64_t vert_cap, int n_flags, int allow_packed, int skip_lo)
 {
     DecompState *st = b.st;
     const int V = st->V;
@@ -109,19 +107,24 @@
         st->n_comp = 0; st->n_vert = 0; st->comp_cap = comp_cap; st->vert_cap = vert_cap;
         st->unsettled = 0; st->overflow = 0; st->bad = 0; st->dead = 0; st->scan_total = 0; st->alive_after = 0;
         st->packed = (allow_packed && b.kc && b.pack_bad && *b.pack_bad == 0) ? 1u : 0u;
+        st->ticket = 0; st->tail_nv = 0; st->tail_ne = 0; st->tail_next = 0;
+        st->refused = (skip_lo && !st->packed) ? 1u : 0u;
+        st->dead = st->refused;
         if (comp_cap >= 0) b.o_off[0] = 0;
     }
 }
 
+template <bool Listed>
 __device__ void ph_round_begin(const DecompBufs &b, Span T, int reset_left)
 {
-    const int V = b.st->V;
-    if (!reset_left && b.st->dead) return;
+    const int V = b.st->V, nv = n_vertices<Listed>(b);
+    if (b.st->refused || (!reset_left && b.st->dead)) return;
     if (T.tid == 0) { b.st->alive_after = 0; if (reset_left) b.st->dead = 0; }
-    const int64_t E = b.st->E;
-    for (int64_t e = T.tid; e < E; e += T.n) b.done[e] = 0;
+    const int64_t E = n_arcs<Listed>(b);
+    for (int64_t j = T.tid; j < E; j += T.n) b.done[arc_at<Listed>(b, j)] = 0;
     const bool packed = b.st->packed != 0;
-    for (int i = T.tid; i < V; i += T.n) {
+    for (int j = T.tid; j < nv; j += T.n) {
+        const int i = vertex_at<Listed>(b, j);
         const int s = i >> 1;
         const int64_t l = reset_left ? 1 : b.left[s];
         if (reset_left && !(i & 1)) b.left[s] = 1;
@@ -142,18 +145,20 @@
 };
 
 
+template <bool Listed>
 __device__ void ph_propose_hi(const DecompBufs &b, Span T, const IterArgs &a)
 {
     if (b.st->dead) return;
     if (a.prev_flag >= 0 && !b.changed[a.prev_flag]) return;
-    const int64_t E = b.st->E;
+    const int64_t E = n_arcs<Listed>(b);
     const int V = b.st->V;
     const int other = (a.parity ^ 1) * V;
     const bool packed = b.st->packed != 0;
-    for (int64_t e = T.tid; e < E; e += T.n) {
+    for (int64_t j = T.tid; j < E; j += T.n) {
+        const int64_t e = arc_at<Listed>(b, j);
         if (b.done[e]) continue;
         const int u = b.src[e], v = b.dst[e];
-        if (b.bi_hi[v] == kClosed) { b.done[e] = 1; continue; }
+        if (slot_word<Listed>(&b.bi_hi[v]) == kClosed) { b.done[e] = 1; continue; }
         const uint64_t k = packed ? (a.stamp_p | b.kc[e]) : (a.stamp | b.khi[e]);
         if (atomicMin(reinterpret_cast<unsigned long long *>(&b.bo_hi[u]), static_cast<unsigned long long>(k)) == kClosed) { b.done[e] = 1; continue; }
         atomicMin(reinterpret_cast<unsigned long long *>(&b.bi_hi[v]), static_cast<unsigned long long>(k));
@@ -161,58 +166,64 @@
     }
 }
 
+template <bool Listed>
 __device__ void ph_propose_lo(const DecompBufs &b, Span T, const IterArgs &a)
 {
     if (b.st->dead) return;
     if (a.prev_flag >= 0 && !b.changed[a.prev_flag]) return;
     if (b.st->packed) return;
-    const int64_t E = b.st->E;
+    const int64_t E = n_arcs<Listed>(b);
     const int mine = a.parity * b.st->V;
-    for (int64_t e = T.tid; e < E; e += T.n) {
+    for (int64_t j = T.tid; j < E; j += T.n) {
+        const int64_t e = arc_at<Listed>(b, j);
         if (b.done[e]) continue;
         const int u = b.src[e], v = b.dst[e];
         const uint64_t k = a.stamp | b.khi[e], lo = b.klo[e];
-        if (b.bo_hi[u] == k) atomicMin(reinterpret_cast<unsigned long long *>(&b.bo_lo[mine + u]), static_cast<unsigned long long>(lo));
-        if (b.bi_hi[v] == k) atomicMin(reinterpret_cast<unsigned long long *>(&b.bi_lo[mine + v]), static_cast<unsigned long long>(lo));
-    }
-}
-
-__device__ void ph_commit_flag(const DecompBufs &b, Span T, const IterArgs &a, volatile unsigned int *took);
-__device__ void ph_commit(const DecompBufs &b, Span T, const IterArgs &a)
-{
-    if (b.st->dead) return;
-    if (a.prev_flag >= 0 && !b.changed[a.prev_flag]) return;
-    ph_commit_flag(b, T, a, b.changed + a.flag);
-}
-__device__ void ph_commit_flag(const DecompBufs &b, Span T, const IterArgs &a, volatile unsigned int *took)
+        if (slot_word<Listed>(&b.bo_hi[u]) == k) atomicMin(reinterpret_cast<unsigned long long *>(&b.bo_lo[mine + u]), static_cast<unsigned long long>(lo));
+        if (slot_word<Listed>(&b.bi_hi[v]) == k) atomicMin(reinterpret_cast<unsigned long long *>(&b.bi_lo[mine + v]), static_cast<unsigned long long>(lo));
+    }
+}
+
+template <bool Listed>
+__device__ bool ph_commit_pass(const DecompBufs &b, Span T, const IterArgs &a)
 {
     bool any = false;
-    const int64_t E = b.st->E;
+    const int64_t E = n_arcs<Listed>(b);
     const int mine = a.parity * b.st->V;
     const bool packed = b.st->packed != 0;
-    for (int64_t e = T.tid; e < E; e += T.n) {
+    for (int64_t j = T.tid; j < E; j += T.n) {
+        const int64_t e = arc_at<Listed>(b, j);
         if (b.done[e]) continue;
         const int u = b.src[e], v = b.dst[e];
         const uint64_t k = packed ? (a.stamp_p | b.kc[e]) : (a.stamp | b.khi[e]);
-        if (b.bo_hi[u] != k || b.bi_hi[v] != k) continue;
+        if (slot_word<Listed>(&b.bo_hi[u]) != k || slot_word<Listed>(&b.bi_hi[v]) != k) continue;
         const uint64_t lo = b.klo[e];
-        if (!a.unique_hi && !packed && (b.bo_lo[mine + u] != lo || b.bi_lo[mine + v] != lo)) continue;
+        if (!a.unique_hi && !packed && (slot_word<Listed>(&b.bo_lo[mine + u]) != lo || slot_word<Listed>(&b.bi_lo[mine + v]) != lo)) continue;
         b.next[u] = v; b.prev[v] = u;
         b.nhi[u] = b.khi[e]; b.nlo[u] = lo;
         b.bo_hi[u] = kClosed; b.bi_hi[v] = kClosed;
         b.done[e] = 1;
         any = true;
     }
-    if (__syncthreads_or(any) && threadIdx.x == 0) *took = 1u;
-}
-
+    return __syncthreads_or(any) != 0;
+}
+__device__ void ph_commit(const DecompBufs &b, Span T, const IterArgs &a)
+{
+    if (b.st->dead) return;
+    if (a.prev_flag >= 0 && !b.changed[a.prev_flag]) return;
+    volatile unsigned int *took = b.changed + a.flag;
+    if (ph_commit_pass<false>(b, T, a) && threadIdx.x == 0) *took = 1u;
+}
+
+template <bool Listed>
 __device__ void ph_heads(const DecompBufs &b, Span T, int round, int last_flag)
 {
     DecompState *st = b.st;
     if (st->dead) return;
     if (T.tid == 0 && last_flag >= 0 && b.changed[last_flag]) st->unsettled = 1;
-    const int V = st->V;
-    for (int v = T.tid; v < V; v += T.n) {
+    const int nv = n_vertices<Listed>(b);
+    for (int j = T.tid; j < nv; j += T.n) {
+        const int v = vertex_at<Listed>(b, j);
         if (!b.alive[v] || b.prev[v] >= 0) continue;
         int len = 0, last = v;
         int64_t least = b.left[v >> 1];
@@ -232,11 +243,13 @@
     }
 }
 
+template <bool Listed>
 __device__ void ph_cycles(const DecompBufs &b, Span T, int round)
 {
-    const int V = b.st->V;
+    const int nv = n_vertices<Listed>(b);
     if (b.st->dead) return;
-    for (int v = T.tid; v < V; v += T.n) {
+    for (int j = T.tid; j < nv; j += T.n) {
+        const int v = vertex_at<Listed>(b, j);
         if (!b.alive[v] || b.on_path[v] == round + 1) continue;
         int len = 1, twin_least = v ^ 1, worst = 0;
         uint64_t whi = b.nhi[v], wlo = b.nlo[v];
@@ -259,13 +272,24 @@
     }
 }
 
+__device__ void ph_round_end(const DecompBufs &b)
+{
+    DecompState *st = b.st;
+    st->dead = __hip_atomic_load(&st->alive_after, __ATOMIC_RELAXED, __HIP_MEMORY_SCOPE_AGENT) == 0;
+    st->n_comp += static_cast<int64_t>(st->scan_total >> 40);
+    st->n_vert += static_cast<int64_t>(st->scan_total & kLenMask);
+    if (st->n_comp <= st->comp_cap) b.o_off[st->n_comp] = st->n_vert;
+}
+
+template <bool Listed>
 __device__ void ph_emit(const DecompBufs &b, Span T, int round, int64_t c0, int64_t v0)
 {
     DecompState *st = b.st;
-    const int V = st->V;
+    const int nv = n_vertices<Listed>(b);
     if (st->dead) return;
     int64_t alive = 0;
-    for (int v = T.tid; v < V; v += T.n) {
+    for (int j = T.tid; j < nv; j += T.n) {
+        const int v = vertex_at<Listed>(b, j);
         const uint64_t la = b.len_a[v];
         if (!la) continue;
         const int64_t len = static_cast<int64_t>(la & kLenMask);
@@ -292,27 +316,129 @@
     if (alive) atomicAdd(&wg_alive, static_cast<unsigned long long>(alive));
     __syncthreads();
     if (threadIdx.x == 0 && wg_alive) atomicAdd(reinterpret_cast<unsigned long long *>(&st->alive_after), wg_alive);
-}
-
-
-__global__ void dec_init_kernel(DecompBufs b, int64_t comp_cap, int64_t vert_cap, int n_flags, int allow_packed) { ph_init(b, whole_grid(), comp_cap, vert_cap, n_flags, allow_packed); }
-__global__ void dec_round_begin_kernel(DecompBufs b, int reset_left) { ph_round_begin(b, whole_grid(), reset_left); }
-__global__ void dec_propose_hi_kernel(DecompBufs b, IterArgs a) { ph_propose_hi(b, whole_grid(), a); }
-__global__ void dec_propose_lo_kernel(DecompBufs b, IterArgs a) { ph_propose_lo(b, whole_grid(), a); }
+    if (Listed) return;
+    if (threadIdx.x == 0) {
+        __threadfence();
+        if (atomicAdd(&st->ticket, 1u) == gridDim.x - 1) {
+            __threadfence();
+            ph_round_end(b);
+            st->ticket = 0;
+        }
+    }
+}
+
+__device__ void ph_tail_scan(const DecompBufs &b, Span T)
+{
+    __shared__ uint64_t part[kMaxWaves];
+    const int nv = b.st->tail_nv;
+    const int lane = T.tid & 63, wv = T.tid >> 6, waves = T.n >> 6;
+    uint64_t carry = 0;
+    for (int base = 0; base < nv; base += T.n) {
+        const int j = base + T.tid;
+        const int v = j < nv ? b.vlist[j] : 0;
+        const uint64_t x = j < nv ? b.len_a[v] : 0;
+        const uint64_t incl = wave_incl_scan(x, lane);
+        if (lane == 63) part[wv] = incl;
+        __syncthreads();
+        uint64_t before = 0, all = 0;
+        for (int w = 0; w < waves; w++) { if (w < wv) before += part[w]; all += part[w]; }
+        if (j < nv) b.pos[v] = carry + before + incl - x;
+        carry += all;
+        __syncthreads();
+    }
+    if (T.tid == 0) b.st->scan_total = carry;
+}
+
+__device__ void ph_tail_reopen(const DecompBufs &b, Span T, bool two_words)
+{
+    const int nv = b.st->tail_nv;
+    for (int j = T.tid; j < nv; j += T.n) {
+        const int v = b.vlist[j];
+        if (slot_word<true>(&b.bo_hi[v]) != kClosed) b.bo_hi[v] = kNoKey;
+        if (slot_word<true>(&b.bi_hi[v]) != kClosed) b.bi_hi[v] = kNoKey;
+        if (two_words) { b.bo_lo[v] = kNoKey; b.bi_lo[v] = kNoKey; }
+    }
+}
+
+__global__ void dec_tail_mark_kernel(DecompBufs b, int cap)
+{
+    DecompState *st = b.st;
+    if (st->dead || st->unsettled) return;
+    const Span T = whole_grid();
+    const int V = st->V;
+    for (int v = T.tid; v < V; v += T.n) b.len_a[v] = b.left[v >> 1] > 0 ? 1 : 0;
+    const int64_t E = st->E;
+    volatile int32_t *n_listed = &st->tail_ne;
+    for (int64_t e = T.tid; e < E; e += T.n) {
+        if (b.left[b.src[e] >> 1] <= 0 || b.left[b.dst[e] >> 1] <= 0) continue;
+        if (*n_listed > cap) continue;
+        const int k = atomicAdd(&st->tail_ne, 1);
+        if (k < cap) b.alist[k] = static_cast<int32_t>(e);
+    }
+}
+
+__global__ void dec_tail_list_kernel(DecompBufs b, int cap)
+{
+    DecompState *st = b.st;
+    if (st->dead || st->unsettled) return;
+    const Span T = whole_grid();
+    const int V = st->V;
+    if (T.tid == 0) st->tail_nv = static_cast<int32_t>(st->scan_total);
+    for (int v = T.tid; v < V; v += T.n) {
+        if (!b.len_a[v]) continue;
+        const uint64_t p = b.pos[v];
+        if (p < static_cast<uint64_t>(cap)) b.vlist[p] = v;
+    }
+}
+
+__global__ __launch_bounds__(kTailBlock) void dec_tail_kernel(DecompBufs b, int t0, int t1, int cap, int unique_hi)
+{
+    DecompState *st = b.st;
+    const Span T{static_cast<int>(threadIdx.x), static_cast<int>(blockDim.x)};
+    const bool nothing = st->dead || st->unsettled;
+    const bool declined = st->tail_nv > cap || st->tail_ne > cap;
+    const bool two_words = !unique_hi && !st->packed;
+    __syncthreads();
+    if (nothing || declined) {
+        if (T.tid == 0) st->tail_next = nothing ? t1 : t0;
+        return;
+    }
+    const IterArgs a{1ull << kStampShift, 1ull << kPackedShift, 0, -1, 0, unique_hi};
+    for (int t = t0; t < t1; t++) {
+        ph_round_begin<true>(b, T, 0);
+        __syncthreads();
+        for (;;) {
+            ph_propose_hi<true>(b, T, a);
+            __syncthreads();
+            if (two_words) { ph_propose_lo<true>(b, T, a); __syncthreads(); }
+            if (!ph_commit_pass<true>(b, T, a)) break;
+            ph_tail_reopen(b, T, two_words);
+            __syncthreads();
+        }
+        ph_heads<true>(b, T, t, -1);
+        __syncthreads();
+        ph_cycles<true>(b, T, t);
+        __syncthreads();
+        ph_tail_scan(b, T);
+        __syncthreads();
+        ph_emit<true>(b, T, t, st->n_comp, st->n_vert);
+        __syncthreads();
+        if (T.tid == 0) ph_round_end(b);
+        __syncthreads();
+        if (st->dead) break;
+    }
+    if (T.tid == 0) st->tail_next = t1;
+}
+
+
+__global__ void dec_init_kernel(DecompBufs b, int64_t comp_cap, int64_t vert_cap, int n_flags, int allow_packed, int skip_lo) { ph_init(b, whole_grid(), comp_cap, vert_cap, n_flags, allow_packed, skip_lo); }
+__global__ void dec_round_begin_kernel(DecompBufs b, int reset_left) { ph_round_begin<false>(b, whole_grid(), reset_left); }
+__global__ void dec_propose_hi_kernel(DecompBufs b, IterArgs a) { ph_propose_hi<false>(b, whole_grid(), a); }
+__global__ void dec_propose_lo_kernel(DecompBufs b, IterArgs a) { ph_propose_lo<false>(b, whole_grid(), a); }
 __global__ void dec_commit_kernel(DecompBufs b, IterArgs a) { ph_commit(b, whole_grid(), a); }
-__global__ void dec_heads_kernel(DecompBufs b, int round, int last_flag) { ph_heads(b, whole_grid(), round, last_flag); }
-__global__ void dec_cycles_kernel(DecompBufs b, int round) { ph_cycles(b, whole_grid(), round); }
-__global__ void dec_emit_kernel(DecompBufs b, int round) { ph_emit(b, whole_grid(), round, b.st->n_comp, b.st->n_vert); }
-
-__global__ void dec_round_end_kernel(DecompBufs b)
-{
-    DecompState *st = b.st;
-    if (blockIdx.x || threadIdx.x || st->dead) return;
-    st->dead = st->alive_after == 0;
-    st->n_comp += static_cast<int64_t>(st->scan_total >> 40);
-    st->n_vert += static_cast<int64_t>(st->scan_total & kLenMask);
-    if (st->n_comp <= st->comp_cap) b.o_off[st->n_comp] = st->n_vert;
-}
+__global__ void dec_heads_kernel(DecompBufs b, int round, int last_flag) { ph_heads<false>(b, whole_grid(), round, last_flag); }
+__global__ void dec_cycles_kernel(DecompBufs b, int round) { ph_cycles<false>(b, whole_grid(), round); }
+__global__ void dec_emit_kernel(DecompBufs b, int round) { ph_emit<false>(b, whole_grid(), round, b.st->n_comp, b.st->n_vert); }
 
 size_t up256(size_t v) { return (v + 255) / 256 * 256; }
 
@@ -347,6 +473,7 @@
     b.alive = c.take<uint8_t>(V); b.kind = c.take<uint8_t>(V);
     b.partials = c.take<uint64_t>(kDecompGrid + 1);
     b.changed = c.take<uint32_t>(static_cast<size_t>(rounds) * static_cast<size_t>(iters));
+    b.vlist = c.take<int32_t>(kTailCapMax); b.alist = c.take<int32_t>(kTailCapMax);
     b.o_off = c.take<int64_t>(static_cast<size_t>(comp_cap) + 1);
     b.o_verts = c.take<int32_t>(static_cast<size_t>(vert_cap));
     b.o_iter = c.take<int32_t>(static_cast<size_t>(comp_cap));
@@ -371,8 +498,7 @@
 int scan_u64(palace_ctx *ctx, const uint64_t *in, uint64_t *out, const int32_t *n_dev, uint64_t *partials, uint64_t *total_dev)
 {
     hipLaunchKernelGGL(scan_partials_kernel, dim3(kDecompGrid), dim3(kDecompBlock), 0, ctx->stream, in, n_dev, partials);
-    hipLaunchKernelGGL(scan_prefix_kernel, dim3(1), dim3(kDecompBlock), 0, ctx->stream, partials, kDecompGrid, total_dev);
-    hipLaunchKernelGGL(scan_apply_kernel, dim3(kDecompGrid), dim3(kDecompBlock), 0, ctx->stream, in, out, n_dev, partials);
+    hipLaunchKernelGGL(scan_apply_kernel, dim3(kDecompGrid), dim3(kDecompBlock), 0, ctx->stream, in, out, n_dev, partials, total_dev);
     PALACE_HIP_TRY(hipGetLastError());
     return PALACE_OK;
 }
@@ -383,14 +509,14 @@
 constexpr int kWideGridDefault = 2048;
 inline dim3 wide_grid(const palace_ctx *ctx) { return dim3(ctx->match_grid > 0 ? ctx->match_grid : kWideGridDefault); }
 
-void enqueue_iterations(palace_ctx *ctx, const DecompBufs &b, int first, int n, uint64_t *count, int flag0, bool unique_hi)
+void enqueue_iterations(palace_ctx *ctx, const DecompBufs &b, int first, int n, uint64_t *count, int flag0, bool unique_hi, bool skip_lo)
 {
     for (int k = 0; k < n; k++) {
         IterArgs a{((1ull << 21) - 1 - *count) << kStampShift, static_cast<uint64_t>((kPackedStamps - 1 - *count) & (kPackedStamps - 1)) << kPackedShift,
                    (first + k) & 1, k ? flag0 + k - 1 : -1, flag0 + k, unique_hi ? 1 : 0};
         (*count)++;
         hipLaunchKernelGGL(dec_propose_hi_kernel, wide_grid(ctx), kBlock, 0, ctx->stream, b, a);
-        if (!unique_hi) hipLaunchKernelGGL(dec_propose_lo_kernel, wide_grid(ctx), kBlock, 0, ctx->stream, b, a);
+        if (!unique_hi && !skip_lo) hipLaunchKernelGGL(dec_propose_lo_kernel, wide_grid(ctx), kBlock, 0, ctx->stream, b, a);
         hipLaunchKernelGGL(dec_commit_kernel, wide_grid(ctx), kBlock, 0, ctx->stream, b, a);
     }
 }
@@ -402,30 +528,31 @@
     int rc = scan_u64(ctx, b.len_a, b.pos, &b.st->V, b.partials, &b.st->scan_total);
     if (rc) return rc;
     hipLaunchKernelGGL(dec_emit_kernel, wide_grid(ctx), kBlock, 0, ctx->stream, b, round);
-    hipLaunchKernelGGL(dec_round_end_kernel, dim3(1), dim3(64), 0, ctx->stream, b);
     PALACE_HIP_TRY(hipGetLastError());
     return PALACE_OK;
 }
 
 }
 
-int decomp_begin(palace_ctx *ctx, const DecompBufs &b, int rounds, int64_t comp_cap, int64_t vert_cap)
+int decomp_begin(palace_ctx *ctx, const DecompBufs &b, DecompRun &run, int rounds, int64_t comp_cap, int64_t vert_cap, bool unique_hi)
 {
     PALACE_REQUIRE(rounds >= 1 && rounds <= kMaxRounds, "round count out of range");
-    static_assert(kDecompGrid <= kDecompBlock, "scan_prefix_kernel scans the block sums with one workgroup");
+    static_assert(kDecompGrid <= kDecompBlock, "scan_apply_kernel adds the chunk sums up with one thread each");
     const int allow_packed = !ctx->match_two_word_keys && static_cast<int64_t>(rounds) * kMaxIters < kPackedStamps ? 1 : 0;
-    hipLaunchKernelGGL(dec_init_kernel, wide_grid(ctx), kBlock, 0, ctx->stream, b, comp_cap, vert_cap, rounds * kMaxIters, allow_packed);
+    run = DecompRun{};
+    run.skip_lo = allow_packed && !unique_hi;
+    hipLaunchKernelGGL(dec_init_kernel, wide_grid(ctx), kBlock, 0, ctx->stream, b, comp_cap, vert_cap, rounds * kMaxIters, allow_packed, run.skip_lo ? 1 : 0);
     PALACE_HIP_TRY(hipGetLastError());
     return PALACE_OK;
 }
 
 int decomp_rounds(palace_ctx *ctx, const DecompBufs &b, int t0, int t1, int rounds, int aggressive, int iters, bool unique_hi,
-                  uint64_t *count)
+                  bool skip_lo, uint64_t *count)
 {
     PALACE_REQUIRE(0 <= t0 && t0 <= t1 && t1 <= rounds && rounds <= kMaxRounds && iters >= 1 && iters <= kMaxIters, "round / iteration count out of range");
     for (int t = t0; t < t1; t++) {
         hipLaunchKernelGGL(dec_round_begin_kernel, wide_grid(ctx), kBlock, 0, ctx->stream, b, (aggressive && t == rounds - 1) ? 1 : 0);
-        enqueue_iterations(ctx, b, 0, iters, count, t * kMaxIters, unique_hi);
+        enqueue_iterations(ctx, b, 0, iters, count, t * kMaxIters, unique_hi, skip_lo);
         int rc = enqueue_read_off(ctx, b, t, t * kMaxIters + iters - 1);
         if (rc) return rc;
     }
@@ -438,13 +565,13 @@
 {
     PALACE_REQUIRE(rounds >= 1 && rounds <= kMaxRounds, "round count out of range");
     constexpr int kBatch = 16;
-    hipLaunchKernelGGL(dec_init_kernel, wide_grid(ctx), kBlock, 0, ctx->stream, b, comp_cap, vert_cap, kBatch, 0);
+    hipLaunchKernelGGL(dec_init_kernel, wide_grid(ctx), kBlock, 0, ctx->stream, b, comp_cap, vert_cap, kBatch, 0, 0);
     uint64_t count = 0;
     for (int t = 0; t < rounds; t++) {
         hipLaunchKernelGGL(dec_round_begin_kernel, wide_grid(ctx), kBlock, 0, ctx->stream, b, (aggressive && t == rounds - 1) ? 1 : 0);
         for (int first = 0;; first += kBatch) {
             PALACE_HIP_TRY(hipMemsetAsync(b.changed, 0, kBatch * sizeof(uint32_t), ctx->stream));
-            enqueue_iterations(ctx, b, first, kBatch, &count, 0, unique_hi);
+            enqueue_iterations(ctx, b, first, kBatch, &count, 0, unique_hi, false);
             uint32_t last = 0;
             PALACE_HIP_TRY(hipMemcpyAsync(&last, b.changed + kBatch - 1, sizeof last, hipMemcpyDeviceToHost, ctx->stream));
             PALACE_HIP_TRY(hipStreamSynchronize(ctx->stream));
@@ -463,14 +590,24 @@
 
 int decomp_group(palace_ctx *ctx, const DecompBufs &b, DecompRun &run, int rounds, int aggressive, bool unique_hi)
 {
-    const int first = kFirstGroupRounds;
-    const int t0 = run.next_round, t1 = std::min(rounds, t0 + (t0 == 0 ? first : kRoundsPerGroup));
+    const int t0 = run.next_round, t1 = std::min(rounds, t0 + (t0 == 0 ? 1 : kRoundsPerGroup));
     for (int t = t0; t < t1; t++) {
         const int iters = ctx->match_iters > 0 ? std::min(ctx->match_iters, kMaxIters) : (t == 0 ? kFirstRoundIters : kLaterRoundIters);
-        int rc = decomp_rounds(ctx, b, t, t + 1, rounds, aggressive, iters, unique_hi, &run.count);
+        int rc = decomp_rounds(ctx, b, t, t + 1, rounds, aggressive, iters, unique_hi, run.skip_lo, &run.count);
         if (rc) return rc;
     }
     run.next_round = t1;
+    const int t_end = aggressive ? rounds - 1 : rounds;
+    if (t0 == 0 && t_end > 1) {
+        const int cap = std::min(ctx->match_tail_cap >= 0 ? ctx->match_tail_cap : kTailCapDefault, kTailCapMax);
+        hipLaunchKernelGGL(dec_tail_mark_kernel, wide_grid(ctx), kBlock, 0, ctx->stream, b, cap);
+        int rc = scan_u64(ctx, b.len_a, b.pos, &b.st->V, b.partials, &b.st->scan_total);
+        if (rc) return rc;
+        hipLaunchKernelGGL(dec_tail_list_kernel, wide_grid(ctx), kBlock, 0, ctx->stream, b, cap);
+        hipLaunchKernelGGL(dec_tail_kernel, dim3(1), dim3(kTailBlock), 0, ctx->stream, b, 1, t_end, cap, unique_hi ? 1 : 0);
+        PALACE_HIP_TRY(hipGetLastError());
+        run.tail_pending = true;
+    }
     return PALACE_OK;
 }
 
@@ -480,7 +617,7 @@
     for (;;) {
         PALACE_HIP_TRY(hipMemcpyAsync(h_state, b.st, sizeof *h_state, hipMemcpyDeviceToHost, ctx->stream));
         PALACE_HIP_TRY(hipStreamSynchronize(ctx->stream));
-        if (h_state->unsettled) {
+        if (h_state->unsettled || h_state->refused) {
             int rc = reset_left();
             if (rc) return rc;
             rc = decomp_run_checked(ctx, b, rounds, aggressive, unique_hi, comp_cap, vert_cap, max_iterations);
@@ -489,6 +626,7 @@
             PALACE_HIP_TRY(hipStreamSynchronize(ctx->stream));
             return PALACE_OK;
         }
+        if (run.tail_pending) { run.next_round = h_state->tail_next; run.tail_pending = false; }
         if (run.next_round >= rounds) return PALACE_OK;
         if (h_state->alive_after == 0) {
             if (!aggressive) return PALACE_OK;
diff --git a/palace_amd/csrc/decomp.hpp b/palace_amd/csrc/decomp.hpp
--- a/palace_amd/csrc/decomp.hpp
+++ b/palace_amd/csrc/decomp.hpp
@@ -20,6 +20,9 @@
 constexpr int kDecompBlock = 256;
 constexpr int kMaxRounds = 1024;
 constexpr int kMaxIters = 64;
+constexpr int kTailCapMax = 1 << 16;
+constexpr int kTailCapDefault = 8192;
+constexpr int kTailBlock = 1024;
 
 struct DecompState {
     int32_t S, V;
@@ -33,6 +36,10 @@
     uint32_t packed;
     uint64_t scan_total;
     int64_t alive_after;
+    uint32_t refused;
+    uint32_t ticket;
+    int32_t tail_nv, tail_ne;
+    int32_t tail_next;
 };
 
 struct DecompBufs {
@@ -53,6 +60,7 @@
     uint8_t *alive = nullptr, *kind = nullptr;
     uint64_t *partials = nullptr;
     uint32_t *changed = nullptr;
+    int32_t *vlist = nullptr, *alist = nullptr;
     int64_t *o_off = nullptr;
     int32_t *o_verts = nullptr, *o_iter = nullptr, *o_open = nullptr;
     uint8_t *o_kind = nullptr;
@@ -60,12 +68,17 @@
 
 size_t decomp_bytes(int64_t s_cap, int64_t e_cap, int64_t comp_cap, int64_t vert_cap, int rounds, int iters);
 void decomp_carve(DecompBufs &b, char *base, int64_t s_cap, int64_t e_cap, int64_t comp_cap, int64_t vert_cap, int rounds, int iters);
-constexpr int kFirstRoundIters = 7, kLaterRoundIters = 4, kRoundsPerGroup = 5, kFirstGroupRounds = 5;
-int decomp_begin(palace_ctx *ctx, const DecompBufs &b, int rounds, int64_t comp_cap, int64_t vert_cap);
+constexpr int kFirstRoundIters = 7, kLaterRoundIters = 4, kRoundsPerGroup = 5;
+struct DecompRun {
+    int next_round = 0;
+    uint64_t count = 0;
+    bool skip_lo = false;
+    bool tail_pending = false;
+};
+int decomp_begin(palace_ctx *ctx, const DecompBufs &b, DecompRun &run, int rounds, int64_t comp_cap, int64_t vert_cap, bool unique_hi);
 int decomp_rounds(palace_ctx *ctx, const DecompBufs &b, int t0, int t1, int rounds, int aggressive, int iters, bool unique_hi,
-                  uint64_t *count);
+                  bool skip_lo, uint64_t *count);
 
-struct DecompRun { int next_round = 0; uint64_t count = 0; };
 int decomp_group(palace_ctx *ctx, const DecompBufs &b, DecompRun &run, int rounds, int aggressive, bool unique_hi);
 int decomp_finish(palace_ctx *ctx, const DecompBufs &b, DecompRun &run, int rounds, int aggressive, bool unique_hi, int64_t comp_cap,
                   int64_t vert_cap, int64_t max_iterations, DecompState *h_state, const std::function<int()> &reset_left);
diff --git a/palace_amd/csrc/filter.hip b/palace_amd/csrc/filter.hip
--- a/palace_amd/csrc/filter.hip
+++ b/palace_amd/csrc/filter.hip
@@ -651,8 +651,7 @@
     s->f.use_paths = use_paths ? 1 : 0;
     int rc = enqueue_match(ctx, s, d_edges, use_paths != 0);
     if (rc) return rc;
-    s->run = DecompRun{};
-    if ((rc = decomp_begin(ctx, s->b, rounds, s->comp_cap, s->vert_cap))) return rc;
+    if ((rc = decomp_begin(ctx, s->b, s->run, rounds, s->comp_cap, s->vert_cap, false))) return rc;
     if ((rc = decomp_group(ctx, s->b, s->run, rounds, s->aggressive, false))) return rc;
     PALACE_HIP_TRY(hipMemcpyAsync(s->h_fs, s->f.fs, sizeof(FilterState), hipMemcpyDeviceToHost, ctx->stream));
     s->rounds = std::max(s->rounds, rounds);
diff --git a/palace_amd/csrc/match.hip b/palace_amd/csrc/match.hip
--- a/palace_amd/csrc/match.hip
+++ b/palace_amd/csrc/match.hip
@@ -244,8 +244,8 @@
     auto fail = [&](int code) { (void)hipStreamSynchronize(st); return code; };
     hipError_t e = hipSuccess;
     if ((rc = upload())) return fail(rc);
-    if ((rc = decomp_begin(ctx, b, rounds, comp_cap, vert_cap))) return fail(rc);
     DecompRun run;
+    if ((rc = decomp_begin(ctx, b, run, rounds, comp_cap, vert_cap, true))) return fail(rc);
     if ((rc = decomp_group(ctx, b, run, rounds, aggressive, true))) return fail(rc);
     auto reset_left = [&]() -> int {
         PALACE_HIP_TRY(hipMemcpyAsync(b.left, p_left, static_cast<size_t>(S) * 8, hipMemcpyHostToDevice, st));
@@ -355,6 +355,9 @@
     } else if (!std::strcmp(name, "one_word_keys")) {
         PALACE_REQUIRE(value == 0 || value == 1, "one_word_keys must be 0 or 1");
         ctx->match_two_word_keys = value == 0;
+    } else if (!std::strcmp(name, "decomp_tail_cap")) {
+        PALACE_REQUIRE(value >= -1 && value <= palace::kTailCapMax, "decomp_tail_cap out of range");
+        ctx->match_tail_cap = static_cast<int>(value);
     } else if (!std::strcmp(name, "decomp_grid")) {
         PALACE_REQUIRE(value >= 0 && value <= 65536, "decomp_grid out of range");
         ctx->match_grid = static_cast<int>(value);
```
